# LilYau350/Variance-Aware-Weight

Hardware: AMD Instinct MI355X
Metric: training images/sec (higher is better)
Workload: dtype bf16; 1 GPU; DiT-B/4, 4x32x32 latents, 1000 classes; Trainer.train_step: q_sample + fwd + lambda-weighted MSE + bwd + AdamW + EMA; global batch 256 = 256 per GPU; global_batch=256, per_gpu_batch=256, parallelism=dp1, weight_type=lambda, hip_graph=False

## Files before the change

include/vaw_hip.h:

```cpp
#ifndef VAW_HIP_H
#define VAW_HIP_H
#include <stdint.h>

#ifdef __cplusplus
extern "C" {
#endif

typedef enum { VAW_OK = 0, VAW_ERR_INVALID = -1, VAW_ERR_LAUNCH = -2, VAW_ERR_UNSUPPORTED = -3 } vaw_status;
typedef enum { VAW_F32 = 0, VAW_BF16 = 1,
               VAW_FP8 = 2, VAW_BF8 = 3 ,
               VAW_F64 = 4  } vaw_dtype;
typedef void* vaw_stream;

int vaw_version(void);
const char* vaw_last_error_string(void);


int vaw_qsample_fwd(const float* x0, const float* noise, const int64_t* t, const float* tab_a, const float* tab_s,
                    int num_timesteps, float* x_t, int B, int64_t per_sample, vaw_stream stream);

int vaw_mix_rows(const float* x, const float* y, const float* ca, const float* cb, float* out, int B,
                 int64_t per_sample, vaw_stream stream);

int vaw_wmse_fwd(const float* model_out, const float* x0, const float* noise, const float* ca, const float* cb,
// ... 95 lines not shown
                        vaw_stream stream);


#define VAW_RESAMPLER_MAX_T 4096

int vaw_resampler_update(const int64_t* ts, const float* losses, int n, int T, int H, double* ring, int64_t* seen, int* bad,
                         vaw_stream stream);

int vaw_resampler_draw(const double* ring, const int64_t* seen, int T, int H, double uniform_prob, const double* u, int B,
                       int64_t* out_t, float* out_w, double* p, vaw_stream stream);


int vaw_row_sqnorms(const float* X, int64_t n, int D, float* out, vaw_stream stream);

int64_t vaw_pairwise_workspace_bytes(int64_t nu, int64_t nv, int k1);
int vaw_pairwise_ksmallest(const float* U, int64_t nu, const float* V, int64_t nv, int D, const float* norm_u, const float* norm_v,
                           int k1, float* out, void* ws, int64_t ws_bytes, vaw_stream stream);

int vaw_ksmallest_merge(const float* parts, int64_t n, int P, int k1, int64_t part_stride, int64_t row_stride, float* out,
                        vaw_stream stream);

int vaw_pairwise_within(const float* U, int64_t nu, const float* V, int64_t nv, int D, const float* norm_u, const float* norm_v,
                        const float* radii_u, int Ku, const float* radii_v, int Kv, uint8_t* u_in, uint8_t* v_in, vaw_stream stream);

int64_t vaw_pairwise_polysum_workspace_bytes(int64_t nu, int64_t nv, int batches);
int vaw_pairwise_polysum(const float* U, int64_t nu, const float* V, int64_t nv, int D, const int32_t* u_idx, const int32_t* v_idx, int batches,
                         double gamma, double coef0, int degree, int skip_diagonal, double* rowsum, void* ws, int64_t ws_bytes,
                         vaw_stream stream);

int64_t vaw_pairwise_count_workspace_bytes(int64_t nu, int64_t nv, int Kv);
int vaw_pairwise_count_within(const float* U, int64_t nu, const float* V, int64_t nv, int D, const float* norm_u, const float* norm_v,
                              const float* radii_v, int Kv, int32_t* u_count, uint8_t* v_in, void* ws, int64_t ws_bytes, vaw_stream stream);

int vaw_col_mean_f64(const float* X, int64_t n, int D, double* mu, vaw_stream stream);
int vaw_cov_f64(const float* X, int64_t n, int D, const double* mu, double* sigma, vaw_stream stream);

int vaw_head_logits(const float* X, int64_t n, int D, const float* Wt, int C, float* logits, int64_t ld, vaw_stream stream);
int vaw_is_rows(const float* in, int64_t n, int C, int64_t ld, int probs, double* lse, double* h, vaw_stream stream);
int vaw_is_colsums(const float* in, const double* lse, int64_t n, int C, int64_t ld, int probs, int64_t row0, int64_t split_size, double* colsum,
                   vaw_stream stream);
int vaw_is_finish(const double* h, const double* colsum, int64_t N, int C, int64_t split_size, double* scores, vaw_stream stream);


typedef struct {
    const float* bias;
    int act;
    const void* aux_in;
    void* aux_out;
    const float* gate;
    int64_t gate_ld;
    const void* resid;
    const float* rowadd;
    int rows_per_batch;
    float alpha;
    float beta;
    int out_f32;
    float* colsum_out;
    float colsum_beta;
    int resid_is_act;
    float* rowsum_a_out;
    float rowsum_a_beta;
    float* colsum_partial_out;
    int64_t* colsum_rows_out;
} vaw_epilogue;

int vaw_gemm(vaw_dtype dt, int a_kmajor, int b_kmajor, int64_t M, int64_t N, int64_t K, const void* A, int64_t lda,
             const void* B, int64_t ldb, void* C, int64_t ldc, const vaw_epilogue* epi_host, float* workspace,
             int64_t workspace_floats, vaw_stream stream);

typedef struct {
    const void* dy;
    const void* x;
    float* dw;
    int64_t M, N, ld_dy, ld_x, ld_dw;
    float alpha;
    int pad_;
    const float* scale_dy;
    const float* scale_x;
} vaw_wgrad_problem;
int64_t vaw_wgrad_grouped_desc_bytes(int n_problems);
int vaw_wgrad_grouped(vaw_dtype dt, int n_problems, const vaw_wgrad_problem* problems, int64_t K, float beta, void* desc_dev,
                      int upload, float* workspace, int64_t workspace_floats, vaw_stream stream);
void vaw_debug_wgrad_engine(int mode);

int64_t vaw_fp8_quantize_workspace_floats(void);
int vaw_fp8_quantize(vaw_dtype src_dt, vaw_dtype dst_format, const void* src, int64_t R, int64_t C, int64_t ld, void* q, int64_t ldq,
                     void* qt, int64_t ldt, float* scale_out, float* workspace, int64_t workspace_floats, vaw_stream stream);
int vaw_fp8_quantize_delayed(vaw_dtype src_dt, vaw_dtype dst_format, const void* src, int64_t R, int64_t C, int64_t ld, void* q,
                             int64_t ldq, void* qt, int64_t ldt, float* state, vaw_stream stream);
int vaw_fp8_scale_update(float* states, int64_t n, vaw_stream stream);
typedef struct {
    const float* src;
    void* q;
    void* qt;
    float* state;
    int64_t R, C, ld, ldq, ldt;
} vaw_fp8_quant_job;
int64_t vaw_fp8_quantize_batched_desc_bytes(int n_jobs);
int vaw_fp8_quantize_delayed_batched(int n_jobs, const vaw_fp8_quant_job* jobs, void* desc_dev, int upload, vaw_stream stream);
int vaw_gemm_fp8(vaw_dtype a_format, int64_t M, int64_t N, int64_t K, const void* A, int64_t lda, const float* scale_a,
                 const void* B, int64_t ldb, const float* scale_b, void* C, int64_t ldc, const vaw_epilogue* epi_host,
                 float* c_fp8_state, vaw_dtype c_fp8_format, float* workspace, int64_t workspace_floats, vaw_stream stream);
int vaw_fp8_transpose(const void* q, int64_t R, int64_t C, int64_t ldq, void* qt, int64_t ldt, vaw_stream stream);

void vaw_p8_set_reserved_cus(int n);
int vaw_gemm_uses_bf16_mfma(vaw_dtype dt, int64_t M, int64_t N, int64_t K, const void* A, int64_t lda, const void* B,
                            int64_t ldb);

typedef struct {
    int tile;
    int force_generic;
    int bk;
    int pd, ws;
    int xcdsplit;
    int sm_max_m, sm_wide_m, sm_nb, sm_stages;
    int ws_loaders;
    int epi, debug;
    int p8_nt, nt_aux;
    int cus;
} vaw_gemm_knobs;
void vaw_gemm_default_knobs(vaw_gemm_knobs* out);
typedef enum {
    VAW_GV_GENERIC = 0,
    VAW_GV_T128_BK32 = 1,
    VAW_GV_T128_BK64 = 2,
    VAW_GV_RING256 = 3,
    VAW_GV_PERSISTENT = 4,
    VAW_GV_SMALL_M = 5,
    VAW_GV_PARKED_DRAIN = 6,
    VAW_GV_WARP_SPEC = 7
} vaw_gemm_variant;
typedef enum { VAW_GR_NONE = 0, VAW_GR_F32 = 1, VAW_GR_BF16 = 2, VAW_GR_F32_ROWSUM = 3 } vaw_gemm_reduce;
typedef enum { VAW_GS_NONE = 0, VAW_GS_FUSED = 1, VAW_GS_SEPARATE = 2 } vaw_gemm_rowsum_mode;
typedef enum { VAW_GC_NONE = 0, VAW_GC_FOLD = 1, VAW_GC_DEFERRED = 2, VAW_GC_SEPARATE = 3 } vaw_gemm_colsum_mode;
typedef struct {
    int variant;
    int ntw;
    int mb, nb, stages;
    int bkt;
    int epi_kind;
    int split;
    int xcd_parts;
    int grid_x, grid_y, grid_z, block;
    int64_t lds_bytes;
    int reduce;
    int rowsum_mode;
    int colsum_mode;
    int64_t colsum_rows;
    int64_t workspace_floats_used;
    int launches;
    int status;
} vaw_gemm_launch;
int vaw_gemm_plan(vaw_dtype dt, int a_kmajor, int b_kmajor, int64_t M, int64_t N, int64_t K, int64_t lda, int64_t ldb,
                  int64_t ldc, int64_t A, int64_t B, int64_t C, const vaw_epilogue* epi_host, int64_t workspace_floats,
                  const vaw_gemm_knobs* knobs, vaw_gemm_launch* out);

typedef struct {
    int epi_kind;
    int a_e5m2;
    int c_fp8, c_e5m2;
    int ntw;
    int tiles_m, tiles_n;
    int nk;
    int split;
    int grid, block;
    int64_t lds_bytes;
// ... 137 lines not shown

int64_t vaw_groupnorm_workspace_floats(int B, int HW, int C);
int vaw_groupnorm_fwd(vaw_dtype dt, const void* x, const float* gamma, const float* beta, const float* scale,
                      const float* shift, int64_t film_ld, int silu, void* y, float* mean, float* rstd, int B, int HW,
                      int C, int G, float eps, float* workspace, vaw_stream stream);
int vaw_groupnorm_apply(vaw_dtype dt, const void* x, const float* mean, const float* rstd, const float* gamma,
                        const float* beta, const float* scale, const float* shift, int64_t film_ld, int silu, void* y, int B,
                        int HW, int C, int G, vaw_stream stream);
int vaw_groupnorm_bwd(vaw_dtype dt, const void* dout, const void* x, const float* mean, const float* rstd,
                      const float* gamma, const float* beta, const float* scale, const float* shift, int64_t film_ld,
                      int silu, const void* dx_add, void* dx, float* dgamma, float* dbeta, float grad_beta, float* dscale,
                      float* dshift, int64_t dfilm_ld, int B, int HW, int C, int G, float* workspace, vaw_stream stream);
typedef enum { VAW_GN_FWD_SUMS = 0, VAW_GN_APPLY = 1, VAW_GN_BWD_SUMS = 2, VAW_GN_BWD_APPLY = 3 } vaw_gn_pass;
typedef enum {
    VAW_GNV_QUAD = 0,
    VAW_GNV_FLAT = 1
} vaw_gn_variant;
typedef struct {
    int variant;
    int rows, nch;
    int nt, rpi;
    int grid_x, grid_y, grid_z, block;
    int64_t lds_bytes;
    int64_t workspace_floats;
    int64_t off_part, off_sums, off_s1, off_s2;
    int status;
} vaw_gn_launch;
int vaw_gn_plan(int pass, vaw_dtype dt, int B, int HW, int C, int G, vaw_gn_launch* out);
int vaw_im2col3x3(vaw_dtype dt, const void* x, void* col, int B, int H, int W, int C, vaw_stream stream);
int vaw_col2im3x3(vaw_dtype dt, const void* dcol, void* dx, int B, int H, int W, int C, vaw_stream stream);
int vaw_conv3x3(vaw_dtype dt, int mode, const void* act, const void* act2, const void* w, void* out, int B, int H, int W,
                int Ci, int Co, const vaw_epilogue* epi_host, float* workspace, int64_t workspace_floats, vaw_stream stream);
typedef enum { VAW_CVR_NONE = 0, VAW_CVR_F32 = 1, VAW_CVR_F32_ROWSUM = 2, VAW_CVR_SLAB_T = 3 } vaw_conv_reduce;
typedef enum { VAW_CVB_NONE = 0, VAW_CVB_FUSED = 1, VAW_CVB_FOLD = 2, VAW_CVB_SEPARATE = 3 } vaw_conv_bias_grad;
typedef struct {
    int variant;
    int ntw;
    int epi_kind;
    int transposed;
    int64_t M, N, K;
    int split;
    int xcd_parts;
    int grid_x, grid_y, block;
    int64_t lds_bytes;
    int reduce;
    int bias_grad;
    int colsum_mode;
    int64_t colsum_rows;
    int64_t workspace_floats_used;
    int launches;
    int status;
} vaw_conv3x3_launch;
int vaw_conv3x3_plan(vaw_dtype dt, int mode, int64_t act, int64_t act2, int64_t w, int64_t out, int B, int H, int W, int Ci, int Co,
                     const vaw_epilogue* epi_host, int64_t workspace, int64_t workspace_floats, const vaw_gemm_knobs* knobs, int cus,
                     vaw_conv3x3_launch* plan);
int64_t vaw_conv3x3_wgrad_small_workspace_floats(int B, int H, int W, int Ci, int Co);
int vaw_conv3x3_wgrad_small(vaw_dtype dt, const void* dy, const void* x, float* dw, float beta, int B, int H, int W, int Ci,
                            int Co, float* workspace, int64_t workspace_floats, vaw_stream stream);
int vaw_resample2(vaw_dtype dt, const void* in, void* out, int B, int Ho, int Wo, int C, int mode, float s,
                  vaw_stream stream);
int vaw_concat_channels(vaw_dtype dt, void* a, void* b, void* cat, int64_t M, int Ca, int Cb, int split,
                        vaw_stream stream);
int vaw_add_inplace(vaw_dtype dt, void* dst, const void* src, int64_t n, vaw_stream stream);
int vaw_mul(vaw_dtype dt, const void* a, const void* b, void* out, int64_t n, vaw_stream stream);
int vaw_subsample2(vaw_dtype dt, const void* in, void* out, int B, int Ho, int Wo, int C, int mode, vaw_stream stream);
int64_t vaw_dropout_bits_words(int64_t n);
int vaw_dropout_pack(vaw_dtype dt, const void* mask, void* bits, int64_t M, int C, vaw_stream stream);
int vaw_dropout_bits_fwd(vaw_dtype dt, const void* x, const void* bits, float keep_scale, void* y, int64_t n, vaw_stream stream);
int vaw_dropout_bits_bwd(vaw_dtype dt, const void* dy, const void* bits, float keep_scale, void* dx, int64_t n, vaw_stream stream);
int vaw_rowvec_add(vaw_dtype dt, void* h, const float* e, int64_t ld, int B, int HW, int C, vaw_stream stream);
int vaw_rowvec_sum(vaw_dtype dt, const void* dh, float* de, int64_t ld, int B, int HW, int C, float beta, vaw_stream stream);
int vaw_nchw_to_nhwc(vaw_dtype dt, const float* nchw, void* nhwc, int B, int C, int HW, vaw_stream stream);
int vaw_nhwc_to_nchw(vaw_dtype dt, const void* nhwc, float* nchw, int B, int C, int HW, vaw_stream stream);


int64_t vaw_sumsq_workspace_floats(void);
int vaw_sumsq(const float* g, int64_t n, float* sumsq_out, int accumulate, float* workspace, vaw_stream stream);
int vaw_adamw_ema_step(float* p, float* g, float* m, float* v, float* ema, void* shadow_bf16, int64_t n, float lr,
                       float beta1, float beta2, float eps, float weight_decay, float bc1, float bc2,
                       float ema_decay, const float* sumsq, float clip_max_norm, int zero_grad, vaw_stream stream);
int vaw_adamw_ema_step_dev(float* p, float* g, float* m, float* v, float* ema, void* shadow_bf16, int64_t n,
                           const float* hyper, float beta1, float beta2, float eps, float weight_decay, float ema_decay,
                           const float* sumsq, float clip_max_norm, int zero_grad, vaw_stream stream);
int vaw_ema_update(float* ema, const float* src, int64_t n, float decay, vaw_stream stream);
int vaw_cast_bf16(const float* src, void* dst, int64_t n, vaw_stream stream);
typedef struct {
    int grid_x, block;
    int rows_per_lane;
    int64_t bytes_read, bytes_written;
} vaw_cast_colsum_launch;
int vaw_cast_colsum_plan(int64_t M, int64_t N, int64_t ld_src, int64_t ld_dst, int64_t src_addr, int64_t dst_addr,
                         int64_t colsum_addr, vaw_cast_colsum_launch* out);
int vaw_cast_colsum_bf16(const float* src, int64_t ld_src, void* dst, int64_t ld_dst, int64_t M, int64_t N, float* colsum,
                         float beta, vaw_stream stream);
int vaw_uncast_bf16(const void* src, float* dst, int64_t n, float scale, vaw_stream stream);

typedef struct {
    int records;
    int colsum_sets;
    int own_dy;
    int Bk;
    int64_t block_bytes;
    int64_t block_stat_bytes;
    int64_t shared_bytes;
    int64_t colsum_bytes;
    int64_t scratch_bytes;
    int64_t cond_bytes;
    int64_t total;
} vaw_dit_ws_plan_t;
int vaw_dit_ws_plan(int dtype, int B, int T, int D, int Dm, int depth, int heads, int Kp, int No, int defer_wgrad, int checkpoint,
                    vaw_dit_ws_plan_t* out);

int vaw_comm_unique_id(void* out128);
int vaw_comm_init(const void* id128, int rank, int world);
int vaw_comm_world(void);
int vaw_comm_destroy(void);
int vaw_allreduce_bucket_start(void* buf, int64_t count, vaw_dtype dt, vaw_stream stream);
int vaw_reduce_scatter_bucket_start(void* buf, int64_t count, vaw_dtype dt, vaw_stream stream);
int vaw_allgather_bucket_start(void* buf, int64_t count, vaw_dtype dt, vaw_stream stream);
int vaw_allreduce_bucket_wait(vaw_stream stream);

#ifdef __cplusplus
}
#endif
#endif
```

variance-aware-weight_amd/_lib.py:

```python
import ctypes as C
import os

import torch

_HERE = os.path.dirname(os.path.abspath(__file__))
LIB_PATH = os.environ.get("VAW_HIP_LIB") or os.path.join(_HERE, "libvaw_hip.so")

F32, BF16, FP8, BF8 = 0, 1, 2, 3
F64 = 4
TORCH_DTYPE = {F32: torch.float32, BF16: torch.bfloat16}

_p, _i, _l, _f, _d = C.c_void_p, C.c_int, C.c_int64, C.c_float, C.c_double


class Epilogue(C.Structure):
    _fields_ = [("bias", _p), ("act", _i), ("aux_in", _p), ("aux_out", _p), ("gate", _p), ("gate_ld", _l),
                ("resid", _p), ("rowadd", _p), ("rows_per_batch", _i), ("alpha", _f), ("beta", _f), ("out_f32", _i),
                ("colsum_out", _p), ("colsum_beta", _f), ("resid_is_act", _i), ("rowsum_a_out", _p), ("rowsum_a_beta", _f),
                ("colsum_partial_out", _p), ("colsum_rows_out", C.POINTER(C.c_int64))]


class AttnDesc(C.Structure):
    _fields_ = [("B", _i), ("H", _i), ("T", _i), ("hd", _i), ("q_sb", _l), ("q_sh", _l), ("q_st", _l), ("q_sd", _l),
                ("o_sb", _l), ("o_sh", _l), ("o_st", _l), ("o_sd", _l), ("scale", _f)]
# ... 75 lines not shown
GN_FWD_SUMS, GN_APPLY, GN_BWD_SUMS, GN_BWD_APPLY = range(4)
GNV_QUAD, GNV_FLAT = range(2)

_PROTOS = {
    "vaw_qsample_fwd": [_p, _p, _p, _p, _p, _i, _p, _i, _l, _p],
    "vaw_mix_rows": [_p, _p, _p, _p, _p, _i, _l, _p],
    "vaw_wmse_fwd": [_p, _p, _p, _p, _p, _p, _p, _i, _l, _p],
    "vaw_wmse_bwd": [_p, _p, _p, _p, _p, _p, _p, _p, _i, _l, _p],
    "vaw_gemm": [_i, _i, _i, _l, _l, _l, _p, _l, _p, _l, _p, _l, C.POINTER(Epilogue), _p, _l, _p],
    "vaw_gemm_uses_bf16_mfma": [_i, _l, _l, _l, _p, _l, _p, _l],
    "vaw_colsum": [_i, _p, _l, _l, _l, _p, _f, _p, _l, _p],
    "vaw_ln_modulate_fwd": [_i, _p, _p, _p, _l, _p, _p, _p, _i, _i, _i, _f, _p],
    "vaw_gate_resid_fwd_contracts": [_i, _i, _i],
    "vaw_gate_resid_ln_modulate_fwd": [_i, _p, _p, _l, _p, _p, _p, _p, _l, _p, _p, _p, _i, _i, _i, _f, _p],
    "vaw_ln_modulate_bwd": [_i, _p, _p, _p, _p, _p, _l, _p, _p, _p, _p, _l, _i, _i, _i, _p, _l, _p],
    "vaw_gate_bwd": [_i, _p, _p, _p, _l, _p, _p, _l, _p, _i, _i, _i, _p, _l, _p],
    "vaw_reduce_rows": [_p, _l, _l, _p, _f, _p],
    "vaw_reduce_rows_batched": [_i, _p, _f, _p, _i, _p],
    "vaw_ln_modulate_bwd_gate": [_i, _p, _p, _p, _p, _p, _l, _p, _p, _p, _p, _l, _p, _p, _p, _p, _p, _i, _i, _i, _p, _l, _p],
    "vaw_ln_modulate_bwd_gate_fp8": [_p, _p, _p, _p, _p, _l, _p, _p, _p, _p, _l, _p, _p, _p, _p, _i, _p, _p, _i, _i, _i, _p, _l, _p],
    "vaw_patchify": [_i, _p, _p, _i, _i, _i, _i, _i, _p],
    "vaw_patchify_bwd": [_p, _p, _i, _i, _i, _i, _i, _p],
    "vaw_unpatchify": [_i, _p, _p, _i, _i, _i, _i, _i, _p],
    "vaw_unpatchify_bwd": [_i, _p, _p, _i, _i, _i, _i, _i, _p],
    "vaw_timestep_embedding": [_i, _p, _p, _i, _i, _f, _p],
    "vaw_silu_fwd": [_i, _p, _p, _l, _p],
    "vaw_silu_bwd": [_p, _p, _p, _l, _p],
    "vaw_add_embedding": [_p, _p, _p, _p, _i, _i, _i, _p],
    "vaw_embedding_bwd": [_p, _p, _p, _i, _i, _i, _f, _p],
    "vaw_attn_fwd": [_i, C.POINTER(AttnDesc), _p, _p, _p, _p, _p, _p],
    "vaw_attn_bwd": [_i, C.POINTER(AttnDesc), _p, _p, _p, _p, _p, _p, _p, _p, _p, _p, _p],
    "vaw_attn_bwd_colsum": [_i, C.POINTER(AttnDesc), _p, _p, _p, _p, _p, _p, _p, _p, _p, _p, _p, C.POINTER(C.c_int64), _p],
    "vaw_comm_unique_id": [_p],
    "vaw_comm_init": [_p, _i, _i],
    "vaw_comm_world": [],
    "vaw_comm_destroy": [],
    "vaw_allreduce_bucket_start": [_p, _l, _i, _p],
    "vaw_reduce_scatter_bucket_start": [_p, _l, _i, _p],
    "vaw_allgather_bucket_start": [_p, _l, _i, _p],
    "vaw_allreduce_bucket_wait": [_p],
    "vaw_groupnorm_fwd": [_i, _p, _p, _p, _p, _p, _l, _i, _p, _p, _p, _i, _i, _i, _i, _f, _p, _p],
    "vaw_groupnorm_apply": [_i, _p, _p, _p, _p, _p, _p, _p, _l, _i, _p, _i, _i, _i, _i, _p],
    "vaw_groupnorm_bwd": [_i, _p, _p, _p, _p, _p, _p, _p, _p, _l, _i, _p, _p, _p, _p, _f, _p, _p, _l, _i, _i, _i, _i, _p, _p],
    "vaw_im2col3x3": [_i, _p, _p, _i, _i, _i, _i, _p],
    "vaw_col2im3x3": [_i, _p, _p, _i, _i, _i, _i, _p],
    "vaw_conv3x3": [_i, _i, _p, _p, _p, _p, _i, _i, _i, _i, _i, C.POINTER(Epilogue), _p, _l, _p],
    "vaw_vb_fwd": [_p, _p, _p, _p, _p, _i, _i, _f, _p, _i, _l, _p],
    "vaw_vb_bwd": [_p, _p, _p, _p, _p, _i, _i, _f, _p, _p, _p, _i, _l, _p],
    "vaw_bpd_terms": [_p, _p, _l, _p, _p, _p, _p, _i, _i, _i, _p, _p, _p, _l, _i, _i, _l, _p],
    "vaw_guided_sample_step": [_i, _p, _p, _p, _p, _l, _f, _p, _p, _p, _i, _i, _i, _f, _p, _p, _p, _p, _i, _l, _p],
    "vaw_cfg_combine": [_p, _p, _l, _f, _p, _i, _l, _p],
    "vaw_finish_images": [_p, _i, _p, _i, _i, _i, _i, _p],
    "vaw_edm_input": [_p, _p, _p, _i, _i, _p, _p, _p, _i, _l, _p],
    "vaw_edm_step": [_i, _i, _p, _p, _l, _f, _p, _p, _p, _i, _i, _p, _p, _p, _i, _l, _p],
    "vaw_dpm_input": [_p, _p, _i, _i, _p, _p, _i, _l, _p],
    "vaw_dpm_step": [_i, _i, _p, _p, _l, _f, _p, _p, _p, _p, _p, _i, _i, _p, _p, _p, _p, _i, _l, _p],
    "vaw_flow_step": [_i, _i, _i, _p, _p, _l, _f, _p, _p, _p, _p, _p, _p, _i, _i, _i, _p, _p, _i, _l, _p],
    "vaw_randn_seeded": [_p, _i, _p, _i, _l, _l, _i, _i, _p],
    "vaw_rk_stage": [_i, _i, _p, _p, _l, _f, _p, _p, _p, _i, _i, _p, C.POINTER(_i), C.POINTER(_f), _i, _f, _p, _p, _p, _f, _f, _p, _l, _i, _l, _p],
    "vaw_rk_scaled_sumsq": [_p, _p, _p, _p, _f, _f, _p, _l, _i, _l, _p],
    "vaw_rk_sumsq_finish": [_p, _l, _p, _p],
    "vaw_flow_logp_stage": [_i, _p, _l, _p, _p, _p, _p, _p, _i, _i, _p, _p, C.POINTER(C.c_double), _i, C.c_double, _p, _p, _p, _l, _i, _l, _p],
    "vaw_flow_logp_prior": [_p, _p, _p, _l, _i, _l, _p],
    "vaw_prior_bpd": [_p, _f, _f, _p, _i, _l, _p],
    "vaw_resampler_update": [_p, _p, _i, _i, _i, _p, _p, _p, _p],
    "vaw_resampler_draw": [_p, _p, _i, _i, C.c_double, _p, _i, _p, _p, _p, _p],
    "vaw_conv3x3_narrow": [_i, _i, _p, _p, _p, _p, _i, _i, _i, _i, _i, _p],
    "vaw_conv3x3_wgrad_small": [_i, _p, _p, _p, _f, _i, _i, _i, _i, _i, _p, _l, _p],
    "vaw_resample2": [_i, _p, _p, _i, _i, _i, _i, _i, _f, _p],
    "vaw_concat_channels": [_i, _p, _p, _p, _l, _i, _i, _i, _p],
    "vaw_add_inplace": [_i, _p, _p, _l, _p],
    "vaw_mul": [_i, _p, _p, _p, _l, _p],
    "vaw_subsample2": [_i, _p, _p, _i, _i, _i, _i, _i, _p],
    "vaw_dropout_pack": [_i, _p, _p, _l, _i, _p],
    "vaw_dropout_bits_fwd": [_i, _p, _p, _f, _p, _l, _p],
    "vaw_dropout_bits_bwd": [_i, _p, _p, _f, _p, _l, _p],
    "vaw_rowvec_add": [_i, _p, _p, _l, _i, _i, _i, _p],
    "vaw_rowvec_sum": [_i, _p, _p, _l, _i, _i, _i, _f, _p],
    "vaw_nchw_to_nhwc": [_i, _p, _p, _i, _i, _i, _p],
    "vaw_nhwc_to_nchw": [_i, _p, _p, _i, _i, _i, _p],
    "vaw_sumsq": [_p, _l, _p, _i, _p, _p],
    "vaw_adamw_ema_step_dev": [_p, _p, _p, _p, _p, _p, _l, _p, _f, _f, _f, _f, _f, _p, _f, _i, _p],
    "vaw_adamw_ema_step": [_p, _p, _p, _p, _p, _p, _l, _f, _f, _f, _f, _f, _f, _f, _f, _p, _f, _i, _p],
    "vaw_ema_update": [_p, _p, _l, _f, _p],
    "vaw_cast_bf16": [_p, _p, _l, _p],
    "vaw_uncast_bf16": [_p, _p, _l, _f, _p],
    "vaw_wgrad_grouped": [_i, _i, _p, _l, _f, _p, _i, _p, _l, _p],
    "vaw_fp8_quantize": [_i, _i, _p, _l, _l, _l, _p, _l, _p, _l, _p, _p, _l, _p],
    "vaw_fp8_quantize_delayed": [_i, _i, _p, _l, _l, _l, _p, _l, _p, _l, _p, _p],
    "vaw_fp8_scale_update": [_p, _l, _p],
    "vaw_fp8_quantize_delayed_batched": [_i, _p, _p, _i, _p],
    "vaw_gemm_fp8": [_i, _l, _l, _l, _p, _l, _p, _p, _l, _p, _p, _l, C.POINTER(Epilogue), _p, _i, _p, _l, _p],
    "vaw_gemm_fp8_plan": [_i, _l, _l, _l, _l, _l, _l, _l, _l, _l, _l, _l, C.POINTER(Epilogue), _l, _i, _l, _l, _i, C.POINTER(GemmFp8Launch)],
    "vaw_fp8_transpose": [_p, _l, _l, _l, _p, _l, _p],
    "vaw_ln_modulate_fwd_fp8": [_p, _p, _p, _l, _p, _p, _i, _p, _p, _i, _i, _i, _f, _p],
    "vaw_gate_bwd_fp8": [_p, _p, _p, _l, _p, _p, _i, _p, _l, _p, _i, _i, _i, _p, _l, _p],
    "vaw_row_plan": [_i, _i, _l, _l, _l, _l, _l, _l, C.POINTER(RowLaunch)],
    "vaw_attn_plan": [_i, _i, C.POINTER(AttnDesc), _l, _l, _l, _l, _l, _l, _l, C.POINTER(AttnLaunch)],
    "vaw_gn_plan": [_i, _i, _i, _i, _i, _i, C.POINTER(GnLaunch)],
    "vaw_gemm_plan": [_i, _i, _i, _l, _l, _l, _l, _l, _l, _l, _l, _l, C.POINTER(Epilogue), _l, C.POINTER(GemmKnobs), C.POINTER(GemmLaunch)],
    "vaw_conv3x3_plan": [_i, _i, _l, _l, _l, _l, _i, _i, _i, _i, _i, C.POINTER(Epilogue), _l, _l, C.POINTER(GemmKnobs), _i, C.POINTER(Conv3x3Launch)],
    "vaw_dit_ws_plan": [_i, _i, _i, _i, _i, _i, _i, _i, _i, _i, _i, C.POINTER(DitWsPlan)],
    "vaw_latent_qsample": [_p, _p, _p, _p, _p, _p, _i, _f, _f, _p, _p, _p, _i, _l, _p],
    "vaw_wmse_fwd_t": [_p, _p, _p, _p, _p, _p, _p, _i, _p, _p, _f, _i, _l, _p],
    "vaw_wmse_bwd_t": [_p, _p, _p, _p, _p, _p, _p, _i, _p, _f, _p, _i, _l, _p],
    "vaw_ln_modulate_bwd_cast": [_i, _p, _p, _p, _p, _p, _l, _p, _p, _p, _p, _l, _i, _i, _i, _p, _l, _p, _p],
    "vaw_silu_bwd_cast": [_p, _p, _p, _p, _l, _p],
    "vaw_cast_colsum_plan": [_l, _l, _l, _l, _l, _l, _l, C.POINTER(CastColsumLaunch)],
    "vaw_cast_colsum_bf16": [_p, _l, _p, _l, _l, _l, _p, _f, _p],
    "vaw_row_sqnorms": [_p, _l, _i, _p, _p],
    "vaw_pairwise_ksmallest": [_p, _l, _p, _l, _i, _p, _p, _i, _p, _p, _l, _p],
    "vaw_ksmallest_merge": [_p, _l, _i, _i, _l, _l, _p, _p],
    "vaw_pairwise_within": [_p, _l, _p, _l, _i, _p, _p, _p, _i, _p, _i, _p, _p, _p],
    "vaw_pairwise_polysum": [_p, _l, _p, _l, _i, _p, _p, _i, _d, _d, _i, _i, _p, _p, _l, _p],
    "vaw_pairwise_count_within": [_p, _l, _p, _l, _i, _p, _p, _p, _i, _p, _p, _p, _l, _p],
    "vaw_col_mean_f64": [_p, _l, _i, _p, _p],
    "vaw_cov_f64": [_p, _l, _i, _p, _p, _p],
    "vaw_head_logits": [_p, _l, _i, _p, _i, _p, _l, _p],
    "vaw_is_rows": [_p, _l, _i, _l, _i, _p, _p, _p],
    "vaw_is_colsums": [_p, _p, _l, _i, _l, _i, _l, _l, _p, _p],
    "vaw_is_finish": [_p, _p, _l, _i, _l, _p, _p],
}

_lib = None


class VawError(RuntimeError):
    pass


def lib():
    global _lib
    if _lib is None:
        if not os.path.exists(LIB_PATH):
            raise VawError(f"{LIB_PATH} not found: build it with `python -c 'import __graft_entry__ as g; g.build()'` "
                           "(there is no CPU fallback for the HIP path)")
        L = C.CDLL(LIB_PATH)
        for name, args in _PROTOS.items():
            if not hasattr(L, name) and os.environ.get("VAW_HIP_LIB"):
                continue
            fn = getattr(L, name)
            fn.argtypes = args
            fn.restype = _i
        L.vaw_version.restype = _i
        L.vaw_last_error_string.restype = C.c_char_p
        L.vaw_colsum_workspace_floats.argtypes = [_l, _l]
        L.vaw_colsum_workspace_floats.restype = _l
        L.vaw_row_bwd_workspace_floats.argtypes = [_i, _i, _i]
        L.vaw_row_bwd_workspace_floats.restype = _l
        L.vaw_conv3x3_wgrad_small_workspace_floats.argtypes = [_i, _i, _i, _i, _i]
        L.vaw_conv3x3_wgrad_small_workspace_floats.restype = _l
        L.vaw_groupnorm_workspace_floats.argtypes = [_i, _i, _i]
        L.vaw_groupnorm_workspace_floats.restype = _l
        if hasattr(L, "vaw_dropout_bits_words"):
            L.vaw_dropout_bits_words.argtypes = [_l]
            L.vaw_dropout_bits_words.restype = _l
        L.vaw_wgrad_grouped_desc_bytes.argtypes = [_i]
        L.vaw_wgrad_grouped_desc_bytes.restype = _l
        L.vaw_reduce_rows_batched_desc_bytes.argtypes = [_i]
        L.vaw_reduce_rows_batched_desc_bytes.restype = _l
        L.vaw_fp8_quantize_batched_desc_bytes.argtypes = [_i]
        L.vaw_fp8_quantize_batched_desc_bytes.restype = _l
        L.vaw_fp8_quantize_workspace_floats.argtypes = []
        L.vaw_fp8_quantize_workspace_floats.restype = _l
        if hasattr(L, "vaw_pairwise_workspace_bytes"):
            L.vaw_pairwise_workspace_bytes.argtypes = [_l, _l, _i]
            L.vaw_pairwise_workspace_bytes.restype = _l
        if hasattr(L, "vaw_pairwise_polysum_workspace_bytes"):
            L.vaw_pairwise_polysum_workspace_bytes.argtypes = [_l, _l, _i]
            L.vaw_pairwise_polysum_workspace_bytes.restype = _l
            L.vaw_pairwise_count_workspace_bytes.argtypes = [_l, _l, _i]
            L.vaw_pairwise_count_workspace_bytes.restype = _l
        if hasattr(L, "vaw_rk_partial_count"):
            L.vaw_rk_partial_count.argtypes = [_i, _l]
            L.vaw_rk_partial_count.restype = _l
        L.vaw_sumsq_workspace_floats.argtypes = []
        L.vaw_sumsq_workspace_floats.restype = _l
        L.vaw_debug_force_rowwise_attention.argtypes = [_i]
        L.vaw_debug_force_rowwise_attention.restype = None
        L.vaw_debug_force_generic_gemm.argtypes = [_i]
        L.vaw_debug_force_generic_gemm.restype = None
        L.vaw_debug_gemm_tile.argtypes = [_i]
        L.vaw_debug_gemm_tile.restype = None
        if hasattr(L, "vaw_gemm_default_knobs"):
            L.vaw_gemm_default_knobs.argtypes = [C.POINTER(GemmKnobs)]
            L.vaw_gemm_default_knobs.restype = None
        if hasattr(L, "vaw_debug_gn_flat"):
            L.vaw_debug_gn_flat.argtypes = [_i]
            L.vaw_debug_gn_flat.restype = None
        L.vaw_p8_set_reserved_cus.argtypes = [_i]
        L.vaw_p8_set_reserved_cus.restype = None
        if hasattr(L, "vaw_debug_wgrad_engine"):
            L.vaw_debug_wgrad_engine.argtypes = [_i]
            L.vaw_debug_wgrad_engine.restype = None
        L.vaw_debug_cu_hog.argtypes = [_i, _i, _p]
        L.vaw_debug_cu_hog.restype = _i
        _lib = L
    return _lib


def exported_symbols():
    return sorted(list(_PROTOS) + ["vaw_version", "vaw_last_error_string", "vaw_colsum_workspace_floats",
                                   "vaw_sumsq_workspace_floats", "vaw_groupnorm_workspace_floats", "vaw_wgrad_grouped_desc_bytes",
                                   "vaw_conv3x3_wgrad_small_workspace_floats", "vaw_row_bwd_workspace_floats",
                                   "vaw_fp8_quantize_workspace_floats", "vaw_p8_set_reserved_cus", "vaw_debug_wgrad_engine", "vaw_reduce_rows_batched_desc_bytes", "vaw_fp8_quantize_batched_desc_bytes",
                                   "vaw_gemm_default_knobs", "vaw_dropout_bits_words", "vaw_pairwise_workspace_bytes", "vaw_rk_partial_count",
                                   "vaw_pairwise_polysum_workspace_bytes", "vaw_pairwise_count_workspace_bytes"])


STEP_FUSED = os.environ.get("VAW_STEP_FUSED", "1") != "0"
ROWS_FWD_FUSED = os.environ.get("VAW_ROWS_FWD_FUSED", "1") != "0"


def check(rc, what):
    if rc != 0:
        raise VawError(f"{what} failed ({rc}): {lib().vaw_last_error_string().decode()}")


def stream_ptr():
    return torch.cuda.current_stream().cuda_stream


def ptr(t):
    return 0 if t is None else t.data_ptr()


def need_cuda(*tensors):
    for t in tensors:
        if t is not None and not t.is_cuda:
            raise VawError("vaw_amd runs on the GPU only: got a CPU tensor (no CPU fallback exists by design)")
```

variance-aware-weight_amd/csrc/elementwise.hip:

```cpp
#include "common.h"

static inline int stream_grid(int64_t work_items, int block) {
    int64_t g = (work_items + block - 1) / block;
    const int64_t cap = 256 * 8;
    return (int)(g < 1 ? 1 : (g > cap ? cap : g));
}

__device__ __forceinline__ void gather_mix_coef(const float* __restrict__ ca, const float* __restrict__ cb, const int64_t* __restrict__ t,
                                                int T, int b, float& a, float& c) {
    const int64_t tt = t[b];
    const bool ok = tt >= 0 && tt < T;
    a = ok ? ca[tt] : __builtin_nanf("");
    c = ok ? cb[tt] : __builtin_nanf("");
}

template <bool GATHER>
__global__ void mix_rows_kernel(const float* __restrict__ x, const float* __restrict__ y, const float* __restrict__ ca,
                                const float* __restrict__ cb, const int64_t* __restrict__ t, int T,
                                float* __restrict__ out, int64_t n) {
    const int b = blockIdx.y;
    float a, c;
    if (GATHER) {
        gather_mix_coef(ca, cb, t, T, b, a, c);
    } else {
// ... 776 lines not shown

__device__ __forceinline__ void adam_one(float& p, float& g, float& m, float& v, float& e, bool has_ema, float gs,
                                         const AdamArgs& a) {
    const float gg = g * gs;
    p = p * (1.f - a.lr * a.wd);
    m = m + (gg - m) * (1.f - a.b1);
    v = v * a.b2 + (1.f - a.b2) * gg * gg;
    const float denom = sqrtf(v) / a.bc2_sqrt + a.eps;
    p = p - (a.lr / a.bc1) * (m / denom);
    if (has_ema) e = e * a.ema_decay + p * (1.f - a.ema_decay);
}

#define ADAM_U 4
__device__ __forceinline__ f32x4 nt_load4(const float* p) { return __builtin_nontemporal_load(reinterpret_cast<const f32x4*>(p)); }
__global__ void __launch_bounds__(256)
adamw_ema_kernel(float* __restrict__ p, float* __restrict__ g, float* __restrict__ m, float* __restrict__ v,
                 float* __restrict__ ema, bf16_t* __restrict__ shadow, int64_t n, const float* __restrict__ sumsq, AdamArgs a,
                 const float* __restrict__ hyper) {
    if (hyper) {
        a.lr = hyper[0];
        a.bc1 = hyper[1];
        a.bc2_sqrt = sqrtf(hyper[2]);
    }
    float gs = 1.f;
    if (a.clip > 0.f) {
        const float coef = a.clip / (sqrtf(*sumsq) + 1e-6f);
        gs = coef < 1.f ? coef : 1.f;
    }
    const int64_t n4 = n / 4;
    const bool has_ema = ema != nullptr;
    constexpr int64_t TILE = (int64_t)ADAM_U * 256;
    const int64_t n_tiles = n4 / TILE;
    for (int64_t t = blockIdx.x; t < n_tiles; t += gridDim.x) {
        const int64_t i0 = t * TILE + threadIdx.x;
        f32x4 pv[ADAM_U], gv[ADAM_U], mv[ADAM_U], vv[ADAM_U], ev[ADAM_U];
#pragma unroll
        for (int u = 0; u < ADAM_U; ++u) {
            const int64_t i = 4 * (i0 + 256 * u);
            pv[u] = nt_load4(p + i); gv[u] = nt_load4(g + i); mv[u] = nt_load4(m + i); vv[u] = nt_load4(v + i);
            ev[u] = has_ema ? nt_load4(ema + i) : f32x4{0, 0, 0, 0};
        }
#pragma unroll
        for (int u = 0; u < ADAM_U; ++u) {
            const int64_t i = 4 * (i0 + 256 * u);
#pragma unroll
            for (int j = 0; j < 4; ++j) {
                float pj = pv[u][j], gj = gv[u][j], mj = mv[u][j], vj = vv[u][j], ej = ev[u][j];
                adam_one(pj, gj, mj, vj, ej, has_ema, gs, a);
                pv[u][j] = pj; mv[u][j] = mj; vv[u][j] = vj; ev[u][j] = ej;
            }
            __builtin_nontemporal_store(pv[u], reinterpret_cast<f32x4*>(p + i));
            __builtin_nontemporal_store(mv[u], reinterpret_cast<f32x4*>(m + i));
            __builtin_nontemporal_store(vv[u], reinterpret_cast<f32x4*>(v + i));
            if (has_ema) __builtin_nontemporal_store(ev[u], reinterpret_cast<f32x4*>(ema + i));
            if (shadow) store4(shadow + i, pv[u]);
            if (a.zero_grad) store4(g + i, f32x4{0, 0, 0, 0});
        }
    }
    for (int64_t i = n_tiles * TILE + blockIdx.x * (int64_t)blockDim.x + threadIdx.x; i < n4; i += (int64_t)gridDim.x * blockDim.x) {
        f32x4 pv = load4(p + 4 * i), gv = load4(g + 4 * i), mv = load4(m + 4 * i), vv = load4(v + 4 * i);
        f32x4 ev = has_ema ? load4(ema + 4 * i) : f32x4{0, 0, 0, 0};
#pragma unroll
        for (int j = 0; j < 4; ++j) {
            float pj = pv[j], gj = gv[j], mj = mv[j], vj = vv[j], ej = ev[j];
            adam_one(pj, gj, mj, vj, ej, has_ema, gs, a);
            pv[j] = pj; mv[j] = mj; vv[j] = vj; ev[j] = ej;
        }
        store4(p + 4 * i, pv);
        store4(m + 4 * i, mv);
        store4(v + 4 * i, vv);
        if (has_ema) store4(ema + 4 * i, ev);
        if (shadow) store4(shadow + 4 * i, pv);
        if (a.zero_grad) store4(g + 4 * i, f32x4{0, 0, 0, 0});
    }
    for (int64_t i = n4 * 4 + blockIdx.x * (int64_t)blockDim.x + threadIdx.x; i < n; i += (int64_t)gridDim.x * blockDim.x) {
        float pv = p[i], gv = g[i], mv = m[i], vv = v[i], ev = has_ema ? ema[i] : 0.f;
        adam_one(pv, gv, mv, vv, ev, has_ema, gs, a);
        p[i] = pv; m[i] = mv; v[i] = vv;
        if (has_ema) ema[i] = ev;
        if (shadow) shadow[i] = (bf16_t)pv;
        if (a.zero_grad) g[i] = 0.f;
    }
}
static inline int adam_grid(int64_t n) {
    const int64_t tiles = n / 4 / (ADAM_U * 256);
    const int64_t cap = 256 * 8;
    return (int)(tiles < 1 ? 1 : (tiles > cap ? cap : tiles));
}

extern "C" int vaw_adamw_ema_step(float* p, float* g, float* m, float* v, float* ema, void* shadow_bf16, int64_t n,
                                  float lr, float beta1, float beta2, float eps, float weight_decay, float bc1,
                                  float bc2, float ema_decay, const float* sumsq, float clip_max_norm, int zero_grad,
                                  vaw_stream stream) {
    VAW_CHECK_ARG(n > 0, "adamw: n<=0");
    VAW_CHECK_ARG((((uintptr_t)p | (uintptr_t)g | (uintptr_t)m | (uintptr_t)v | (uintptr_t)ema) & 15) == 0 &&
                      ((uintptr_t)shadow_bf16 & 7) == 0, "adamw: buffers must be 16-byte aligned");
    VAW_CHECK_ARG(clip_max_norm <= 0.f || sumsq != nullptr, "adamw: clip needs sumsq");
    AdamArgs a{lr, beta1, beta2, eps, weight_decay, bc1, sqrtf(bc2), ema_decay, clip_max_norm, zero_grad};
    adamw_ema_kernel<<<adam_grid(n), 256, 0, (hipStream_t)stream>>>(p, g, m, v, ema, (bf16_t*)shadow_bf16, n, sumsq, a, nullptr);
    VAW_CHECK_LAUNCH("adamw_ema");
    return VAW_OK;
}

extern "C" int vaw_adamw_ema_step_dev(float* p, float* g, float* m, float* v, float* ema, void* shadow_bf16, int64_t n,
                                      const float* hyper, float beta1, float beta2, float eps, float weight_decay,
                                      float ema_decay, const float* sumsq, float clip_max_norm, int zero_grad,
                                      vaw_stream stream) {
    VAW_CHECK_ARG(n > 0 && hyper, "adamw_dev: n<=0 or no hyper buffer");
    VAW_CHECK_ARG((((uintptr_t)p | (uintptr_t)g | (uintptr_t)m | (uintptr_t)v | (uintptr_t)ema) & 15) == 0 &&
                      ((uintptr_t)shadow_bf16 & 7) == 0, "adamw_dev: buffers must be 16-byte aligned");
    VAW_CHECK_ARG(clip_max_norm <= 0.f || sumsq != nullptr, "adamw_dev: clip needs sumsq");
    AdamArgs a{0.f, beta1, beta2, eps, weight_decay, 1.f, 1.f, ema_decay, clip_max_norm, zero_grad};
    adamw_ema_kernel<<<adam_grid(n), 256, 0, (hipStream_t)stream>>>(p, g, m, v, ema, (bf16_t*)shadow_bf16, n, sumsq, a, hyper);
    VAW_CHECK_LAUNCH("adamw_ema_dev");
    return VAW_OK;
}

__global__ void ema_kernel(float* __restrict__ ema, const float* __restrict__ src, int64_t n, float d) {
    for (int64_t i = blockIdx.x * (int64_t)blockDim.x + threadIdx.x; i < n; i += (int64_t)gridDim.x * blockDim.x)
        ema[i] = ema[i] * d + src[i] * (1.f - d);
}
extern "C" int vaw_ema_update(float* ema, const float* src, int64_t n, float decay, vaw_stream stream) {
    VAW_CHECK_ARG(n > 0, "ema: n<=0");
    ema_kernel<<<stream_grid(n, 256), 256, 0, (hipStream_t)stream>>>(ema, src, n, decay);
    VAW_CHECK_LAUNCH("ema");
    return VAW_OK;
}

__global__ void cast_bf16_kernel(const float* __restrict__ src, bf16_t* __restrict__ dst, int64_t n) {
    const int64_t n4 = n / 4;
    for (int64_t i = blockIdx.x * (int64_t)blockDim.x + threadIdx.x; i < n4; i += (int64_t)gridDim.x * blockDim.x)
        store4(dst + 4 * i, load4(src + 4 * i));
    for (int64_t i = n4 * 4 + blockIdx.x * (int64_t)blockDim.x + threadIdx.x; i < n; i += (int64_t)gridDim.x * blockDim.x)
        dst[i] = (bf16_t)src[i];
}
extern "C" int vaw_cast_bf16(const float* src, void* dst, int64_t n, vaw_stream stream) {
    VAW_CHECK_ARG(n > 0 && ((uintptr_t)src & 15) == 0 && ((uintptr_t)dst & 7) == 0, "cast_bf16: n<=0 or unaligned");
    cast_bf16_kernel<<<stream_grid(n / 4 + 1, 256), 256, 0, (hipStream_t)stream>>>(src, (bf16_t*)dst, n);
    VAW_CHECK_LAUNCH("cast_bf16");
    return VAW_OK;
}

__global__ void uncast_bf16_kernel(const bf16_t* __restrict__ src, float* __restrict__ dst, int64_t n, float scale) {
    const int64_t n8 = n / 8;
    for (int64_t i = blockIdx.x * (int64_t)blockDim.x + threadIdx.x; i < n8; i += (int64_t)gridDim.x * blockDim.x) {
        const bf16x8 v = reinterpret_cast<const bf16x8*>(src)[i];
        f32x4 a = {(float)v[0], (float)v[1], (float)v[2], (float)v[3]}, b = {(float)v[4], (float)v[5], (float)v[6], (float)v[7]};
        reinterpret_cast<f32x4*>(dst)[2 * i] = a * scale;
        reinterpret_cast<f32x4*>(dst)[2 * i + 1] = b * scale;
    }
    for (int64_t i = n8 * 8 + blockIdx.x * (int64_t)blockDim.x + threadIdx.x; i < n; i += (int64_t)gridDim.x * blockDim.x)
        dst[i] = scale * (float)src[i];
}
extern "C" int vaw_uncast_bf16(const void* src, float* dst, int64_t n, float scale, vaw_stream stream) {
    VAW_CHECK_ARG(n > 0 && ((uintptr_t)src & 15) == 0 && ((uintptr_t)dst & 15) == 0, "uncast_bf16: n<=0 or unaligned");
    uncast_bf16_kernel<<<stream_grid(n / 8 + 1, 256), 256, 0, (hipStream_t)stream>>>((const bf16_t*)src, dst, n, scale);
    VAW_CHECK_LAUNCH("uncast_bf16");
    return VAW_OK;
}

__global__ void latent_qsample_kernel(const float* __restrict__ latent, const float* __restrict__ eps, const float* __restrict__ noise,
                                      const int64_t* __restrict__ t, const float* __restrict__ tab_a, const float* __restrict__ tab_s,
                                      int T, float scale, float t_scale, float* __restrict__ x0, float* __restrict__ x_t,
                                      float* __restrict__ tf, int64_t n) {
    const int b = blockIdx.y;
    float a, c;
    gather_mix_coef(tab_a, tab_s, t, T, b, a, c);
    if (tf && blockIdx.x == 0 && threadIdx.x == 0) tf[b] = (float)t[b] * t_scale;
    const float* mr = latent + (int64_t)b * 2 * n;
    const float* sr = mr + n;
    const float* er = eps + (int64_t)b * n;
    const float* nr = noise + (int64_t)b * n;
    float* xr = x0 + (int64_t)b * n;
    float* orow = x_t + (int64_t)b * n;
    const int64_t n4 = ((n & 3) == 0) ? n / 4 : 0;
    for (int64_t i = blockIdx.x * (int64_t)blockDim.x + threadIdx.x; i < n4; i += (int64_t)gridDim.x * blockDim.x) {
        const f32x4 x = (load4(mr + 4 * i) + load4(sr + 4 * i) * load4(er + 4 * i)) * scale;
        store4(xr + 4 * i, x);
        store4(orow + 4 * i, a * x + c * load4(nr + 4 * i));
    }
    for (int64_t i = n4 * 4 + blockIdx.x * (int64_t)blockDim.x + threadIdx.x; i < n; i += (int64_t)gridDim.x * blockDim.x) {
        const float x = (mr[i] + sr[i] * er[i]) * scale;
        xr[i] = x;
        orow[i] = a * x + c * nr[i];
    }
}

extern "C" int vaw_latent_qsample(const float* latent, const float* eps, const float* noise, const int64_t* t, const float* tab_a,
                                  const float* tab_s, int num_timesteps, float latent_scale, float t_scale, float* x0, float* x_t,
                                  float* t_float, int B, int64_t per_sample, vaw_stream stream) {
    VAW_CHECK_ARG(B > 0 && B <= 65535 && per_sample > 0 && num_timesteps > 0, "latent_qsample: bad sizes B=%d n=%ld", B, (long)per_sample);
    VAW_CHECK_ARG(latent && eps && noise && t && tab_a && tab_s && x0 && x_t, "latent_qsample: null pointer");
    VAW_CHECK_ARG(per_sample % 4 != 0 || ((((uintptr_t)latent | (uintptr_t)eps | (uintptr_t)noise | (uintptr_t)x0 | (uintptr_t)x_t) & 15) == 0),
                  "latent_qsample: tensors must be 16-byte aligned");
    int gx = stream_grid(per_sample / 4 + 1, 256);
    dim3 grid(gx > 64 ? 64 : gx, B);
    latent_qsample_kernel<<<grid, 256, 0, (hipStream_t)stream>>>(latent, eps, noise, t, tab_a, tab_s, num_timesteps, latent_scale, t_scale,
// ... 100 lines not shown
```

variance-aware-weight_amd/csrc/gemm_p8.hip:

```cpp
#include "gemm_p8_kernel.h"
#include "gemm_plan.h"
static_assert(P8Cfg<3>::lds_bytes == vaw_lds_p8(3) && P8Cfg<4>::lds_bytes == vaw_lds_p8(4), "gemm_plan.h: LDS size of the persistent kernel");

void p8_launch_fwd(const P8Launch& L, const EpiDev& e, hipStream_t s);
void p8_launch_dgrad(const P8Launch& L, const EpiDev& e, hipStream_t s);
void p8_launch_wgrad(const P8Launch& L, const EpiDev& e, hipStream_t s);
void p8_launch_tn(const P8Launch& L, const EpiDev& e, hipStream_t s);

static int g_p8_reserved = 0;
extern "C" void vaw_p8_set_reserved_cus(int n) { g_p8_reserved = n > 0 ? n : 0; }
static int p8_num_cus() {
    static int n = 0, env_r = 0;
    if (!n) {
        int dev = 0;
        hipDeviceProp_t prop;
        if (hipGetDevice(&dev) == hipSuccess && hipGetDeviceProperties(&prop, dev) == hipSuccess) n = prop.multiProcessorCount;
        if (n <= 0) n = 256;
        const char* v = getenv("VAW_P8_RESERVE_CUS");
        env_r = v ? atoi(v) : 0;
    }
    const int r = env_r > g_p8_reserved ? env_r : g_p8_reserved;
    return (r > 0 && r < n - 8) ? n - r : n;
}

int vaw_p8_cus_available() { return p8_num_cus(); }

static double p8_cost(int64_t M, int64_t N, int ntw, int split, int cus) {
    const int bn = 64 * ntw;
    const int64_t items = ((M + 255) / 256) * ((N + bn - 1) / bn) * split;
    const int64_t rounds = (items + cus - 1) / cus;
    return (double)rounds * (ntw == 4 ? 1.0 : 0.85) / split;
}

P8Plan vaw_p8_plan(int64_t M, int64_t N, int64_t K, bool plain_f32, bool want_colsum, int64_t ws_floats, int force, int cus) {
    P8Plan pl{false, 4, 1, 0};
    if (force == 0) return pl;
    const int nk = (int)(K / 64);
    double best = 1e30;
    for (int ntw = 4; ntw >= 3; --ntw) {
        if (force == 2 && ntw != 4) continue;
        if (force == 3 && ntw != 3) continue;
        const int bn = 64 * ntw;
        const int64_t tiles = ((M + 255) / 256) * ((N + bn - 1) / bn);
        if (ntw == 3 && force != 3) {
            const int64_t pad4 = ((N + 255) / 256) * 256, pad3 = ((N + 191) / 192) * 192;
            if (pad3 > pad4) continue;
        }
        int smax = 1;
        if (plain_f32 && !want_colsum && ws_floats > 0) {
            int64_t s = nk / 4;
            if (s > ws_floats / (M * N)) s = ws_floats / (M * N);
            if (s > 64) s = 64;
            if (s > cus / tiles) s = cus / tiles;
            smax = s < 1 ? 1 : (int)s;
        }
        for (int s = 1; s <= smax; ++s) {
            const int per = (nk + s - 1) / s;
            if ((nk + per - 1) / per != s) continue;
            double c = p8_cost(M, N, ntw, s, cus) * nk;
            if (s > 1) c += 3.0;
            if (c < best - 1e-9) { best = c; pl.ntw = ntw; pl.split = s; }
        }
    }
    const int bn = 64 * pl.ntw;
    const int64_t items = ((M + 255) / 256) * ((N + bn - 1) / bn) * pl.split;
    pl.grid = (int)(items < cus ? items : cus);
    pl.use = force > 0 || (items >= cus / 2 && nk / pl.split >= 4 && M >= 256 && N >= 128);
    return pl;
}

void vaw_p8_launch(const P8Plan& pl, int epi, int a_kmajor, int b_kmajor, int64_t M, int64_t N, int64_t K, const bf16_t* a, int64_t lda,
                   const bf16_t* b, int64_t ldb, const EpiDev& e, hipStream_t s) {
    const int bn = 64 * pl.ntw;
    const int tiles_m = (int)((M + 255) / 256), tiles_n = (int)((N + bn - 1) / bn), nk = (int)(K / 64);
    static int team_pct = -1;
    if (team_pct < 0) { const char* v = getenv("VAW_P8_TEAM_PCT"); team_pct = v ? atoi(v) : 0; }
    const int64_t items = (int64_t)tiles_m * tiles_n * pl.split;
    const int nk_item = (nk + pl.split - 1) / pl.split;
    const int team_delay = (team_pct > 0 && items >= 2 * pl.grid) ? (int)(nk_item * 160LL * pl.ntw / 4 * team_pct / 100) : 0;
    P8Launch L{a, b, lda, ldb, nk, tiles_m, tiles_n, pl.split, pl.grid, pl.ntw, epi, team_delay};
    if (a_kmajor && b_kmajor) p8_launch_fwd(L, e, s);
    else if (a_kmajor && !b_kmajor) p8_launch_dgrad(L, e, s);
    else if (!a_kmajor && !b_kmajor) p8_launch_wgrad(L, e, s);
    else p8_launch_tn(L, e, s);
}

#include <vector>

void vaw_p8_group_fp8(int ntw, bool a_e5m2, int nk, int grid, const EpiDev& e, const P8Prob* probs_dev, const P8Group& grp, hipStream_t s);
void vaw_g4_launch_group(int nk, int grid, const EpiDev& e, const P8Prob* probs_dev, const P8Group& grp, hipStream_t s);

#define G4_BY_SHAPE 1
static int g_wgrad_engine = -2;
static int wgrad_engine() {
    if (g_wgrad_engine == -2) {
        const char* v = getenv("VAW_WGRAD_ENGINE");
        const int m = v ? atoi(v) : -1;
        g_wgrad_engine = (m == 0 || m == 1) ? m : -1;
    }
    return g_wgrad_engine;
}
extern "C" void vaw_debug_wgrad_engine(int mode) { g_wgrad_engine = (mode == 0 || mode == 1) ? mode : -1; }

extern "C" int64_t vaw_wgrad_grouped_desc_bytes(int n_problems) { return (int64_t)n_problems * (int64_t)sizeof(P8Prob); }

extern "C" int vaw_wgrad_grouped(vaw_dtype dt, int n_problems, const vaw_wgrad_problem* problems, int64_t K, float beta,
                                 void* desc_dev, int upload, float* workspace, int64_t workspace_floats, vaw_stream stream) {
    VAW_CHECK_ARG(dt == VAW_BF16 || dt == VAW_FP8 || dt == VAW_BF8, "wgrad_grouped: bf16 or fp8 operands (the f32 parity mode runs vaw_gemm per layer)");
    const bool f8 = dt == VAW_FP8 || dt == VAW_BF8;
    const int kt = f8 ? 128 : 64;
    VAW_CHECK_ARG(n_problems > 0 && problems && desc_dev && K > 0 && K % kt == 0, "wgrad_grouped: bad arguments (K %% %d)", kt);
    bool all192 = true, any_not256 = false;
    for (int i = 0; i < n_problems; ++i) {
        const vaw_wgrad_problem& q = problems[i];
        VAW_CHECK_ARG(q.dy && q.x && q.dw && q.M >= 16 && q.N >= 16 && q.M % 8 == 0 && q.N % 8 == 0, "wgrad_grouped: problem %d: M, N", i);
        if (f8) VAW_CHECK_ARG(q.ld_dy >= K && q.ld_x >= K && q.ld_dw >= q.N && q.ld_dy % 16 == 0 && q.ld_x % 16 == 0 && q.ld_dw % 4 == 0,
                              "wgrad_grouped: problem %d: leading dimensions (fp8: dy^T [M][K], x^T [N][K])", i);
        else VAW_CHECK_ARG(q.ld_dy >= q.M && q.ld_x >= q.N && q.ld_dw >= q.N && q.ld_dy % 8 == 0 && q.ld_x % 8 == 0 && q.ld_dw % 4 == 0,
                           "wgrad_grouped: problem %d: leading dimensions", i);
        VAW_CHECK_ARG((((uintptr_t)q.dy | (uintptr_t)q.x | (uintptr_t)q.dw) & 15) == 0, "wgrad_grouped: problem %d: alignment", i);
        VAW_CHECK_ARG(q.M < (1 << 30) && q.N < (1 << 30), "wgrad_grouped: problem %d too large", i);
        all192 = all192 && q.N % 192 == 0;
        any_not256 = any_not256 || q.N % 256 != 0;
    }
    const int ntw = (all192 && any_not256) ? 3 : 4, bn = 64 * ntw;
    static thread_local std::vector<P8Prob> host;
    host.resize(n_problems);
    int64_t t_total = 0;
    for (int i = 0; i < n_problems; ++i) {
        const vaw_wgrad_problem& q = problems[i];
        P8Prob& h = host[i];
        h.a = (const bf16_t*)q.dy; h.b = (const bf16_t*)q.x; h.c = q.dw;
        h.lda = q.ld_dy; h.ldb = q.ld_x; h.ldc = q.ld_dw;
        h.M = (int)q.M; h.N = (int)q.N;
        h.alpha = q.alpha != 0.f ? q.alpha : 1.f;
        h.pad_ = 0;
        h.scale_a = f8 ? q.scale_dy : nullptr;
        h.scale_b = f8 ? q.scale_x : nullptr;
        h.tiles_n = (int)((q.N + bn - 1) / bn);
        h.tile0 = (int)t_total;
        t_total += ((q.M + 255) / 256) * h.tiles_n;
        VAW_CHECK_ARG(t_total < (1 << 30), "wgrad_grouped: too many tiles");
    }
    hipStream_t s = (hipStream_t)stream;
    if (upload) {
        const hipError_t rc = vaw_upload_table(desc_dev, host.data(), sizeof(P8Prob) * n_problems, s);
        VAW_CHECK_ARG(rc == hipSuccess, "wgrad_grouped: descriptor upload failed: %s", hipGetErrorString(rc));
    }
    const int cus = p8_num_cus(), nk = (int)(K / kt);
    P8Group grp{};
    grp.n_prob = n_problems;
    grp.t_full = (int)(t_total / cus) * cus;
    grp.t_rem = (int)(t_total - grp.t_full);
    grp.n_split = 1;
    grp.slab = workspace;
    if (grp.t_rem > 0) {
        int64_t sp = cus / grp.t_rem;
        if (sp > nk / 4) sp = nk / 4;
        const int64_t per_split = (int64_t)grp.t_rem * 256 * bn;
        if (workspace_floats <= 0 || !workspace) sp = 0;
        else if (sp > workspace_floats / per_split) sp = workspace_floats / per_split;
        if (sp < 2) {
            grp.t_full = (int)t_total;
            grp.t_rem = 0;
        } else {
            const int per = (nk + (int)sp - 1) / (int)sp;
            grp.n_split = (nk + per - 1) / per;
        }
    }
    const int64_t items = grp.t_full + (int64_t)grp.t_rem * grp.n_split;
    const int grid = (int)(items < cus ? items : cus);
    EpiDev e{};
    e.alpha = 1.f;
    e.beta = beta;
    e.out_f32 = 1;
    e.rpb = 1;
    e.nt_off = 1;
    {
        static int dbg = -1;
        if (dbg < 0) { const char* v = getenv("VAW_GEMM_DEBUG"); dbg = v ? atoi(v) : 0; }
        e.debug = dbg;
    }
    if (f8) vaw_p8_group_fp8(ntw, dt == VAW_BF8, nk, grid, e, (const P8Prob*)desc_dev, grp, s);
    else if (ntw == 4) {
        const int eng = wgrad_engine();
        if (eng == 1 || (eng < 0 && G4_BY_SHAPE)) vaw_g4_launch_group(nk, grid, e, (const P8Prob*)desc_dev, grp, s);
        else p8_launch_group<4>(nk, grid, e, (const P8Prob*)desc_dev, grp, s);
    } else p8_launch_group<3>(nk, grid, e, (const P8Prob*)desc_dev, grp, s);
    if (grp.t_rem > 0) {
        if (ntw == 4) p8_group_fixup_kernel<256><<<grp.t_rem * 8, 256, 0, s>>>((const P8Prob*)desc_dev, grp, beta);
        else p8_group_fixup_kernel<192><<<grp.t_rem * 8, 256, 0, s>>>((const P8Prob*)desc_dev, grp, beta);
    }
    VAW_CHECK_LAUNCH("wgrad_grouped");
    return VAW_OK;
}
```

variance-aware-weight_amd/csrc/gemm_p8_kernel.h:

```cpp
#pragma once
#include <stdlib.h>

#include "gemm_epi.h"

typedef __attribute__((address_space(3))) void* lds_ptr_t;
typedef const __attribute__((address_space(1))) void* gbl_ptr_t;

#ifdef P8_TIMING
#define P8_TS(v) const uint64_t v = __builtin_readcyclecounter()
#define P8_TACC(tA, tB, tC, tD, tE)                                                                       \
    do { tacc[0] += tB - tA; tacc[1] += tC - tB; tacc[2] += tD - tC; tacc[3] += tE - tD; tacc[5] += 1;     \
         if (tprev) tacc[4] += tA - tprev; tprev = tE; } while (0)
#else
#define P8_TS(v) do { } while (0)
#define P8_TACC(tA, tB, tC, tD, tE) do { } while (0)
#endif

#ifndef P8_LATE_AT
#define P8_LATE_AT 2
#endif
#ifndef P8_PH2
#define P8_PH2 0
#endif
#ifndef P8_EPI_PD
// ... 768 lines not shown
    }
    if (NOBR) asm volatile("s_waitcnt vmcnt(0)" ::: "memory");
#ifdef P8_TIMING
    if (blockIdx.x == 0 && lane == 0 && (wid == 0 || wid == 4)) {
        __builtin_amdgcn_s_waitcnt(0);
        uint64_t* out = reinterpret_cast<uint64_t*>((char*)e.C + (int64_t)(wid == 4 ? 128 : 0) * e.ldc * (e.out_f32 ? 4 : 2));
        for (int i = 0; i < 6; ++i) out[i] = tacc[i];
    }
#endif
}


template <bool AK, bool BKM, int NTW, int EPI, int CONV>
static void p8_launch_conv(const bf16_t* a, int64_t lda, const bf16_t* b, int64_t ldb, int nk, int tiles_m, int tiles_n, int split,
                           int grid, const EpiDev& e, const P8Conv& cg, hipStream_t s) {
    static bool attr_done = false;
    const int lds = P8Cfg<NTW>::lds_bytes;
    if (!attr_done) {
        (void)hipFuncSetAttribute((const void*)gemm_p8_kernel<AK, BKM, NTW, EPI, false, CONV>, hipFuncAttributeMaxDynamicSharedMemorySize, lds);
        attr_done = true;
    }
    gemm_p8_kernel<AK, BKM, NTW, EPI, false, CONV><<<grid, 512, lds, s>>>(a, lda, b, ldb, nk, tiles_m, tiles_n, split, e, 0, nullptr, P8Group{}, cg);
}

template <int NTW, int EPI, int F8>
static void p8_launch_fp8_one(const void* a, int64_t lda, const void* b, int64_t ldb, int nk, int tiles_m, int tiles_n, int split, int grid,
                              const EpiDev& e, hipStream_t s) {
    static bool attr_done = false;
    const int lds = P8Cfg<NTW>::lds_bytes;
    if (!attr_done) {
        (void)hipFuncSetAttribute((const void*)gemm_p8_kernel<true, true, NTW, EPI, false, 0, F8>, hipFuncAttributeMaxDynamicSharedMemorySize, lds);
        attr_done = true;
    }
    gemm_p8_kernel<true, true, NTW, EPI, false, 0, F8><<<grid, 512, lds, s>>>((const bf16_t*)a, lda, (const bf16_t*)b, ldb, nk, tiles_m, tiles_n,
                                                                               split, e, 0, nullptr, P8Group{}, P8Conv{});
}

template <bool AK, bool BKM, int NTW, int EPI>
static void p8_launch_one(const bf16_t* a, int64_t lda, const bf16_t* b, int64_t ldb, int nk, int tiles_m, int tiles_n, int split,
                          int grid, const EpiDev& e, hipStream_t s, int team_delay) {
    static bool attr_done = false;
    const int lds = P8Cfg<NTW>::lds_bytes;
    if (!attr_done) {
        (void)hipFuncSetAttribute((const void*)gemm_p8_kernel<AK, BKM, NTW, EPI, false, 0>, hipFuncAttributeMaxDynamicSharedMemorySize, lds);
        attr_done = true;
    }
    gemm_p8_kernel<AK, BKM, NTW, EPI, false, 0><<<grid, 512, lds, s>>>(a, lda, b, ldb, nk, tiles_m, tiles_n, split, e, team_delay);
}

template <int NTW, int F8 = 0>
static void p8_launch_group(int nk, int grid, const EpiDev& e, const P8Prob* probs_dev, const P8Group& grp, hipStream_t s) {
    static bool attr_done = false;
    const int lds = P8Cfg<NTW>::lds_bytes;
    if (!attr_done) {
        (void)hipFuncSetAttribute((const void*)gemm_p8_kernel<F8 != 0, F8 != 0, NTW, P8_WGRAD, true, 0, F8>, hipFuncAttributeMaxDynamicSharedMemorySize, lds);
        attr_done = true;
    }
    gemm_p8_kernel<F8 != 0, F8 != 0, NTW, P8_WGRAD, true, 0, F8><<<grid, 512, lds, s>>>(nullptr, 0, nullptr, 0, nk, 0, 0, 1, e, 0, probs_dev, grp, P8Conv{});
}

template <int BN>
__global__ void p8_group_fixup_kernel(const P8Prob* __restrict__ probs, P8Group grp, float beta) {
    const int r = blockIdx.x >> 3, band = blockIdx.x & 7, g = grp.t_full + r;
    int pi = 0;
    while (pi + 1 < grp.n_prob && probs[pi + 1].tile0 <= g) ++pi;
    const P8Prob pr = probs[pi];
    const int tile = g - pr.tile0, tm = tile / pr.tiles_n, tn = tile - tm * pr.tiles_n;
    const int64_t m0 = (int64_t)tm * P8_BM + 32 * band, n0 = (int64_t)tn * BN;
    constexpr int C4 = BN / 4;
    for (int i = threadIdx.x; i < 32 * C4; i += blockDim.x) {
        const int row = i / C4, c4 = (i - row * C4) * 4;
        const int64_t m = m0 + row, n = n0 + c4;
        if (m >= pr.M || n >= pr.N) continue;
        f32x4 acc = {0, 0, 0, 0};
        for (int sp = 0; sp < grp.n_split; ++sp)
            acc += load4(grp.slab + ((int64_t)sp * grp.t_rem + r) * (P8_BM * BN) + (int64_t)(32 * band + row) * BN + c4);
        float* c = pr.c + m * pr.ldc + n;
        acc *= pr.alpha * (pr.scale_a ? *pr.scale_a : 1.f) * (pr.scale_b ? *pr.scale_b : 1.f);
        if (beta != 0.f) acc += beta * load4(c);
        store4(c, acc);
    }
}

struct P8Launch {
    const bf16_t *a, *b;
    int64_t lda, ldb;
    int nk, tiles_m, tiles_n, split, grid, ntw, epi, team_delay;
};
#define P8_CASE(AKv, BKv, EPIv)                                                                                                  \
    case EPIv:                                                                                                                  \
        if (L.ntw == 4) p8_launch_one<AKv, BKv, 4, EPIv>(L.a, L.lda, L.b, L.ldb, L.nk, L.tiles_m, L.tiles_n, L.split, L.grid, e, s, L.team_delay); \
        else p8_launch_one<AKv, BKv, 3, EPIv>(L.a, L.lda, L.b, L.ldb, L.nk, L.tiles_m, L.tiles_n, L.split, L.grid, e, s, L.team_delay);           \
        break
```

variance-aware-weight_amd/dit.py:

```python
import os

import numpy as np
import torch
import torch.nn as nn

from . import _lib as L
from . import ops
from ._lib import BF16, F32, ptr
from .flat import FlatModule

__all__ = ["DiT", "DiT_S", "DiT_B", "DiT_L", "DiT_XL", "DiT_models"]


def _sincos_1d(dim, pos):
    omega = 1.0 / 10000 ** (np.arange(dim // 2, dtype=np.float64) / (dim / 2.0))
    ang = np.einsum("m,d->md", pos.reshape(-1), omega)
    return np.concatenate([np.sin(ang), np.cos(ang)], axis=1)


def get_2d_sincos_pos_embed(dim, grid_size):
    gh = np.arange(grid_size, dtype=np.float32)
    gw = np.arange(grid_size, dtype=np.float32)
    grid = np.stack(np.meshgrid(gw, gh), axis=0).reshape([2, 1, grid_size, grid_size])
    return np.concatenate([_sincos_1d(dim // 2, grid[0]), _sincos_1d(dim // 2, grid[1])], axis=1)
# ... 130 lines not shown
            cps = dict(fc2=ops.ColsumPartial(B, D, dev), proj=ops.ColsumPartial(B, D, dev),
                       fc1=ops.ColsumPartial((M + 63) // 64, m.Dm, dev), qkv=ops.ColsumPartial(max(B, M // 64), 3 * D, dev))
            cps["fc2"].rows.value = cps["proj"].rows.value = B
            self._bufs += [c.buf for c in cps.values()]
            return cps

        self.cp = [cp_set()] * Lyr if ckpt else [cp_set() for _ in range(Lyr)]
        if not (ckpt and plan.own_dy):
            self.dyb = e(M, D)
        self.delta = e(B * m.num_heads * T, dtype=f32)
        self.dmod, self.dmod_a = e(B, m.mod_cols, dtype=f32), z(m.mod_cols)
        self.dcs, self.dc, self.dc_a = e(B, D, dtype=f32), e(B, D, dtype=f32), z(D)
        self.dh1s, self.dh1, self.dh1_a = e(B, D, dtype=f32), e(B, D, dtype=f32), z(D)
        self.dxp = e(M, m.Kp, dtype=f32)
        if not self.fp8 and self.nbytes() != plan.total:
            raise L.VawError(f"DiT workspace: allocated {self.nbytes()} bytes, vaw_dit_ws_plan says {plan.total}")

    def nbytes(self):
        return sum(t.numel() * t.element_size() for t in self._bufs)


class _DiTFn(torch.autograd.Function):
    @staticmethod
    def forward(ctx, anchor, model, x, t, y):
        out = model._forward_impl(x, t, y)
        ctx.model, ctx.gen, ctx.need_dx = model, model._ws_cur.gen, x.requires_grad
        ctx.only_dx = bool(model._input_grad_only)
        ctx.x_shape = x.shape
        return out

    @staticmethod
    def backward(ctx, dout):
        m = ctx.model
        if m._ws_cur.gen != ctx.gen:
            raise L.VawError("DiT backward: activations were overwritten by a later forward of the same batch size")
        if m._ws_cur.ckpt != bool(m.activation_checkpointing):
            raise L.VawError("DiT backward: activation_checkpointing was switched between this forward and its backward "
                             "(the workspace of the forward was laid out for the other mode)")
        if bool(m._input_grad_only) != ctx.only_dx:
            raise L.VawError("DiT backward: input_grad_only() was entered or left between this forward and its backward")
        dx = m._backward_impl(dout.contiguous(), ctx.need_dx, ctx.only_dx)
        return (None if L.STEP_FUSED else torch.zeros_like(m._anchor)), None, dx, None, None


class DiT(FlatModule):
    def __init__(self, image_size=32, patch_size=2, in_channels=4, hidden_size=1152, depth=28, num_heads=16,
                 mlp_ratio=4.0, class_dropout_prob=0.1, num_classes=1000, learn_sigma=False, learn_align=False,
                 encoder_depth=8, z_dims=768, projector_dim=2048, compute_dtype="bf16", activation_checkpointing=False):
        super().__init__()
        if learn_align:
            raise NotImplementedError("learn_align (REPA feature alignment) is outside the hot path (SURVEY §2.1 row 12)")
        assert hidden_size % num_heads == 0 and hidden_size % 4 == 0
        self.learn_sigma, self.learn_align = learn_sigma, learn_align
        self.in_channels = in_channels
        self.out_channels = in_channels * 2 if learn_sigma else in_channels
        self.patch_size, self.num_heads, self.depth = patch_size, num_heads, depth
        self.image_size = image_size
        self.encoder_depth = encoder_depth
        self.x_embedder = _PatchEmbed(image_size, patch_size, in_channels, hidden_size)
        self.t_embedder = _TimestepEmbedder(hidden_size)
        self.y_embedder = _LabelEmbedder(num_classes, hidden_size, class_dropout_prob)
        self.pos_embed = nn.Parameter(torch.zeros(1, self.x_embedder.num_patches, hidden_size), requires_grad=False)
        self.blocks = nn.ModuleList([_Block(hidden_size, num_heads, mlp_ratio) for _ in range(depth)])
        self.projectors = None
        self.final_layer = _FinalLayer(hidden_size, patch_size, self.out_channels)
        self.initialize_weights()
        self.D, self.T = hidden_size, self.x_embedder.num_patches
        self.Dm = int(hidden_size * mlp_ratio)
        self.Kp = in_channels * patch_size * patch_size
        self.No = patch_size * patch_size * self.out_channels
        self.mod_cols = (6 * depth + 2) * hidden_size
        self.fp8_grad_format = "e5m2"
        self.fp8_scaling, self.fp8_margin = "delayed", 2.0
        self.fp8_fuse_epilogue = os.environ.get("VAW_FP8_FUSE", "1") != "0"
        self.fp8_fuse_rows = os.environ.get("VAW_FP8_FUSE_ROWS", "1") != "0"
        self._fp8_w, self._fp8_epoch, self._fp8_wstates, self._fp8_wgroup = {}, None, None, None
        self.activation_checkpointing = False
        self.set_compute_dtype(compute_dtype)
        self._anchor = torch.zeros(1, requires_grad=True)
        self._ws, self._ws_cur = {}, None
        self.set_activation_checkpointing(activation_checkpointing)
        self._ckpt_debug_hook = None
        self.grad_ready_hook = None
        self.defer_wgrad = True

    def initialize_weights(self):
        def basic(mod):
            if isinstance(mod, nn.Linear):
                nn.init.xavier_uniform_(mod.weight)
                if mod.bias is not None:
                    nn.init.constant_(mod.bias, 0)
        self.apply(basic)
        pe = get_2d_sincos_pos_embed(self.pos_embed.shape[-1], int(self.x_embedder.num_patches ** 0.5))
        self.pos_embed.data.copy_(torch.from_numpy(pe).float().unsqueeze(0))
        w = self.x_embedder.proj.weight.data
        nn.init.xavier_uniform_(w.view([w.shape[0], -1]))
        nn.init.constant_(self.x_embedder.proj.bias, 0)
        nn.init.normal_(self.y_embedder.embedding_table.weight, std=0.02)
        nn.init.normal_(self.t_embedder.mlp[0].weight, std=0.02)
        nn.init.normal_(self.t_embedder.mlp[2].weight, std=0.02)
        for blk in self.blocks:
            nn.init.constant_(blk.adaLN_modulation[-1].weight, 0)
            nn.init.constant_(blk.adaLN_modulation[-1].bias, 0)
        nn.init.constant_(self.final_layer.adaLN_modulation[-1].weight, 0)
        nn.init.constant_(self.final_layer.adaLN_modulation[-1].bias, 0)
        nn.init.constant_(self.final_layer.linear.weight, 0)
        nn.init.constant_(self.final_layer.linear.bias, 0)

    def set_compute_dtype(self, name):
        name = {"float32": "fp32", "f32": "fp32", "bfloat16": "bf16", "float8": "fp8"}.get(name, name)
        if name not in ("bf16", "fp32", "fp8"):
            raise ValueError(f"compute_dtype must be 'bf16', 'fp32' or 'fp8', got {name}")
        if name == "fp8" and (self.D % 128 or self.Dm % 128):
            raise ValueError("compute_dtype='fp8' needs hidden and MLP widths that are multiples of 128 (one fp8 MFMA K tile)")
        if name == "fp8" and getattr(self, "activation_checkpointing", False):
            raise ValueError(self._CKPT_FP8)
        if name != getattr(self, "compute_dtype", name):
            self.require_fresh_masters("set_compute_dtype()")
        self.compute_dtype = name
        self._dt = F32 if name == "fp32" else BF16
        self._fp8 = name == "fp8"
        self._fp8_w, self._fp8_epoch, self._fp8_wstates, self._fp8_wgroup = {}, None, None, None
        self._ws = {}

    _ONLY_DX_FP8 = ("input_grad_only() does not combine with compute_dtype='fp8': the delayed-scaling state of the fp8 tensors would "
                    "move during an evaluation")

    _CKPT_FP8 = ("activation_checkpointing does not combine with compute_dtype='fp8': re-running a block's forward would update its "
                 "delayed-scaling state twice per step, and the per-block transposed fp8 copies would have to be shared too")

    def set_activation_checkpointing(self, on):
        on = bool(on)
        if on and self._fp8:
            raise ValueError(self._CKPT_FP8)
        self.activation_checkpointing = on
        self._ws = {}

    def _flat_groups(self):
        ada_w = [f"blocks.{i}.adaLN_modulation.1.weight" for i in range(self.depth)] + ["final_layer.adaLN_modulation.1.weight"]
        ada_b = [f"blocks.{i}.adaLN_modulation.1.bias" for i in range(self.depth)] + ["final_layer.adaLN_modulation.1.bias"]
        return [ada_w, ada_b]

    def _apply(self, fn, recurse=True):
        r = super()._apply(fn, recurse)
        self._anchor = fn(self._anchor.detach()).requires_grad_(True)
        self._ws = {}
        return r

    def grad_stage_bounds(self):
        self.ensure_flat()
        off = lambda n: self._flat_offsets[n][0]
        first = [off(f"blocks.{l}.attn.qkv.weight") for l in range(self.depth)] + [off("final_layer.linear.weight")]
        b = {self.depth + 1: (first[-1], self._flat_n_train), 0: (0, first[0])}
        for l in range(self.depth):
            b[l + 1] = (first[l], first[l + 1])
        half = self._ada_split_block()
        if half is not None:
            D = self.D
            wo, bo = off("blocks.0.adaLN_modulation.1.weight"), off("blocks.0.adaLN_modulation.1.bias")
            we = sum(self._flat_offsets["final_layer.adaLN_modulation.1.weight"])
            be = sum(self._flat_offsets["final_layer.adaLN_modulation.1.bias"])
            assert we - wo == (6 * self.depth + 2) * D * D and be - bo == (6 * self.depth + 2) * D
            cut_w, cut_b = wo + 6 * half * D * D, bo + 6 * half * D
            b["ada_hi"] = [(cut_w, we), (cut_b, be)]
            lo = [(0, cut_w), (we, cut_b), (be, first[0])] if wo < bo else [(0, cut_b), (be, cut_w), (we, first[0])]
            b[0] = [r for r in lo if r[1] > r[0]]
        return b

    def _ada_split_block(self):
        return self.depth // 2 if self.depth >= 4 else None

    def unpatchify(self, x):
        c, p = self.out_channels, self.patch_size
        h = w = int(x.shape[1] ** 0.5)
        assert h * w == x.shape[1]
        x = x.float().contiguous()
        img = torch.empty(x.shape[0], c, h * p, w * p, device=x.device, dtype=torch.float32)
        L.check(L.lib().vaw_unpatchify(F32, ptr(x), ptr(img), x.shape[0], c, h * p, w * p, p, L.stream_ptr()), "vaw_unpatchify")
        return img

    def forward(self, x, t, y, **kwargs):
        L.need_cuda(x, t, y)
        if self._input_grad_only and self._fp8:
            raise ValueError(self._ONLY_DX_FP8)
        out = _DiTFn.apply(self._anchor, self, x, t, y)
        return out, None

    stagewise_weight_waits = True

    def _need(self, stage):
        z = getattr(self, "_zero", None)
        if z is not None:
            z.wait_stage(stage)

    def _w(self, name):
        o, _ = self._flat_offsets[name]
        return self._wbase + o * self._wsize

    def _g(self, name):
        o, _ = self._flat_offsets[name]
        return self._gbase + 4 * o

    def _p32(self, name):
        o, _ = self._flat_offsets[name]
        return self._flat.data_ptr() + 4 * o

    def _prepare(self, B):
        self.ensure_flat()
        if self._dt == BF16:
            sh = self.shadow_bf16()
            self._wbase, self._wsize = sh.data_ptr(), 2
        else:
            self._wbase, self._wsize = self._flat.data_ptr(), 4
        adt = L.TORCH_DTYPE[self._dt]
        if self._fp8:
            if (B * self.T) % 128:
                raise L.VawError("compute_dtype='fp8': batch * tokens must be a multiple of 128 (K tile of the weight gradients)")
            self._refresh_fp8_weights()
        key = (B, adt, self._fp8, bool(self.activation_checkpointing), bool(self.defer_wgrad))
        if key not in self._ws:
            self._ws[key] = _Workspace(self, B, adt)
        self._ws_cur = ws = self._ws[key]
        if ws.fp8:
            delayed = self.fp8_scaling == "delayed"
            ws.d_fwd, ws.d_bwd = delayed and ws.calib_fwd, delayed and ws.calib_bwd
            if ws.d_fwd or ws.d_bwd:
                ops.fp8_scale_update(ws.fp8_states)
        return ws

    _FP8_LINEARS = (("attn.qkv.", 3, 1), ("attn.proj.", 1, 1), ("mlp.fc1.", 0, 1), ("mlp.fc2.", 1, 0))

    def _refresh_fp8_weights(self):
        epoch = (self._weights_epoch, self._flat.data_ptr())
        if self._fp8_epoch == epoch:
            return
        self.require_fresh_masters("re-quantising the fp8 weights")
        dev = self._flat.device
        if self._fp8_wstates is None or self._fp8_wstates.device != dev:
            self._fp8_wstates, self._fp8_w, self._fp8_wgroup = ops.fp8_states([L.FP8] * (4 * self.depth), dev, self.fp8_margin), {}, None
        delayed = self.fp8_scaling == "delayed" and bool(self._fp8_w)
        if delayed:
            ops.fp8_scale_update(self._fp8_wstates)
            grp = getattr(self, "_fp8_wgroup", None)
            if grp is None or grp[0] != self._flat.data_ptr():
                pairs = [(self._p32(f"blocks.{l}.{nm}weight"), self._fp8_w[f"blocks.{l}.{nm}weight"])
                         for l in range(self.depth) for nm, _, _ in self._FP8_LINEARS]
                grp = self._fp8_wgroup = (self._flat.data_ptr(), ops.Fp8QuantGroup(pairs, dev))
            grp[1].launch()
            self._fp8_epoch = epoch
            return
# ... 141 lines not shown

    def _attn_desc(self, B):
        d = getattr(self, "_adesc", None)
        if d is None or d.B != B:
            d = self._adesc = ops.attn_desc_token_major(B, self.num_heads, self.T, self.D // self.num_heads)
        return d

    def _wgrad(self, dt, name, dy, x, Nw, Kw, M, beta, bias=True):
        ops.gemm(dt, 0, 0, Nw, Kw, M, dy, Nw, x, Kw, self._g(name + "weight"), Kw, beta=beta, out_f32=True,
                 rowsum_a_out=self._g(name + "bias") if bias else None, rowsum_a_beta=beta)

    def _adaln_wgrad(self, dt, ws, r0, nrows, B, beta):
        D, ld = self.D, self.mod_cols
        gw, gb = self._g("blocks.0.adaLN_modulation.1.weight") + 4 * r0 * D, self._g("blocks.0.adaLN_modulation.1.bias") + 4 * r0
        fused = False
        if dt == BF16:
            dmod_a, es = ptr(ws.dmod_a), 2
            fused = L.STEP_FUSED and ops.cast_colsum_plan(B, nrows, ld, ld, ptr(ws.dmod) + 4 * r0, dmod_a + es * r0, gb) is not None
            if fused:
                ops.cast_colsum(ptr(ws.dmod) + 4 * r0, ld, dmod_a + es * r0, ld, B, nrows, gb, beta)
            else:
                ops.cast_bf16(ws.dmod, ws.dmod_a)
        else:
            dmod_a, es = ptr(ws.dmod), 4
        ops.gemm(dt, 0, 0, nrows, D, ws.Bk, dmod_a + es * r0, ld, ptr(ws.cs), D, gw, D, beta=beta, out_f32=True)
        if not fused:
            ops.colsum(dt, dmod_a + es * r0, B, nrows, ld, gb, beta)
        return dmod_a

    def _backward_impl(self, dout, need_dx, only_dx=False):
        ws = self._ws_cur
        B = ws.B
        dt, D, T, Dm, Lyr, ld = self._dt, self.D, self.T, self.Dm, self.depth, self.mod_cols
        M, lib, st = B * T, L.lib(), L.stream_ptr()
        H = W = self.image_size
        if only_dx:
            if ws.fp8:
                raise ValueError(self._ONLY_DX_FP8)
            beta, self._gbase, hook = 0.0, None, None
        else:
            beta = 1.0 if self.grads_live() else 0.0
            self._gbase = self.flat_grads().data_ptr()
            hook = self.grad_ready_hook
        ada_half = self._ada_split_block() if hook else None
        dres, dD, dDm, dmod = ptr(ws.dres), ptr(ws.dD), ptr(ws.dDm), ptr(ws.dmod)
        mod = ptr(ws.mod)
        es = self._wsize
        defer = ws.defer and dt == BF16
        fp8 = ws.fp8
        own_dy = defer and not fp8
        ckpt = ws.ckpt
        fuse_rows = fp8 and ws.d_bwd and self.fp8_fuse_epilogue and self.fp8_fuse_rows and M % 64 == 0 and D % 128 == 0
        fuse_tail = L.STEP_FUSED and dt == BF16

        def ln_bwd_and_gate(dout_p, x_p, mean_p, rstd_p, scale_p, dres_in, dsh, dsc, nxt, dx_act=0):
            if nxt is None:
                ops.ln_modulate_bwd(dt, dout_p, x_p, mean_p, rstd_p, scale_p, ld, dres_in, dres, dsh, dsc, ld, B, T, D, dx_act=dx_act)
                return
            l2, which = nxt
            nb = ws.blk[l2]
            mo2, dmo2 = mod + 4 * (6 * l2 * D), dmod + 4 * (6 * l2 * D)
            gcol = 5 if which == "mlp" else 2
            y, cp = (nb["y2"], ws.cp[l2]["fc2"]) if which == "mlp" else (nb["y1"], ws.cp[l2]["proj"])
            if fuse_rows:
                ops.ln_modulate_bwd_gate_fp8(dout_p, x_p, mean_p, rstd_p, scale_p, ld, dres_in, dres, dsh, dsc, ld, ptr(y),
                                             mo2 + 4 * gcol * D, nb["f_dy2" if which == "mlp" else "f_dy1"], dmo2 + 4 * gcol * D,
                                             B, T, D, cp.buf.data_ptr())
            else:
                dy = ptr(nb["dy2" if which == "mlp" else "dy1"]) if own_dy else ptr(ws.dyb)
                ops.ln_modulate_bwd_gate(dt, dout_p, x_p, mean_p, rstd_p, scale_p, ld, dres_in, dres, dsh, dsc, ld, ptr(y),
                                         mo2 + 4 * gcol * D, dy, dmo2 + 4 * gcol * D, B, T, D, cp.buf.data_ptr())

        L.check(lib.vaw_unpatchify_bwd(dt, ptr(dout), ptr(ws.dotok), B, self.out_channels, H, W, self.patch_size, st), "unpatchify_bwd")
        if not only_dx:
            self._wgrad(dt, "final_layer.linear.", ptr(ws.dotok), ptr(ws.xf), self.No, D, M, beta)
        ops.gemm(dt, 1, 0, M, D, self.No, ptr(ws.dotok), self.No, self._w("final_layer.linear.weight"), D, dD, D)
        mo, dmo = mod + 4 * (6 * Lyr * D), dmod + 4 * (6 * Lyr * D)
        ln_bwd_and_gate(dD, ptr(ws.xres[2 * Lyr]), ptr(ws.meanf), ptr(ws.rstdf), mo + 4 * D, 0, dmo, dmo + 4 * D,
                        (Lyr - 1, "mlp") if (Lyr and not ckpt) else None)
        if hook:
            hook(Lyr + 1)
        pending = []
        group_cut = Lyr // 2 if (hook and Lyr >= 4) else 0

        def fold_bias(blocks, qkv_too):
            key = (blocks[0], blocks[-1], self._gbase, qkv_too)
            cps = []
            for l in blocks:
                cp, pre = ws.cp[l], f"blocks.{l}."
                names = [("fc2", "mlp.fc2."), ("fc1", "mlp.fc1."), ("proj", "attn.proj.")] + ([("qkv", "attn.qkv.")] if qkv_too else [])
                cps += [(cp[key_cp], pre + nm) for key_cp, nm in names]
            rows = tuple(int(cp.rows.value) for cp, _ in cps)
            ent = ws.bias_groups.get(key)
            if ent is None or ent[1] != rows:
                jobs = [(cp.buf.data_ptr(), self._g(nm + "bias"), r, cp.N) for (cp, nm), r in zip(cps, rows)]
                ent = ws.bias_groups[key] = (ops.ReduceGroup(jobs, dout.device), rows)
            grp = ent[0]
            grp.launch(beta)

        def flush():
            if not pending:
                return
            key = (pending[0], pending[-1], self._gbase)
            grp = ws.wgrad_groups.get(key)
            if grp is None:
                probs = []
                for l in pending:
                    b, pre = ws.blk[l], f"blocks.{l}."
                    if fp8:
                        for name, fdy, fx, Nw, Kw in ((pre + "mlp.fc2.", b["f_dy2"], b["f_a"], D, Dm), (pre + "mlp.fc1.", b["f_dhid"], b["f_xm2"], Dm, D),
                                                      (pre + "attn.proj.", b["f_dy1"], b["f_ao"], D, D), (pre + "attn.qkv.", b["f_dqkv"], b["f_xm"], 3 * D, D)):
                            probs.append((ptr(fdy.qt), ptr(fx.qt), self._g(name + "weight"), Nw, Kw, M, M, Kw, 0.0, 0, ptr(fdy.scale), ptr(fx.scale)))
                        continue
                    for name, dy, x, Nw, Kw in ((pre + "mlp.fc2.", b["dy2"], b["a"], D, Dm), (pre + "mlp.fc1.", b["dDm"], b["xm2"], Dm, D),
                                                (pre + "attn.proj.", b["dy1"], b["ao"], D, D), (pre + "attn.qkv.", b["dqkv"], b["xm"], 3 * D, D)):
                        probs.append((ptr(dy), ptr(x), self._g(name + "weight"), Nw, Kw, Nw, Kw, Kw))
                grp = ws.wgrad_groups[key] = ops.WgradGroup(probs, M, dout.device)
            grp.launch((L.BF8 if self.fp8_grad_format == "e5m2" else L.FP8) if fp8 else dt, beta)
            fold_bias(list(pending), True)
            if hook:
                for l in pending:
                    hook(l + 1)
            pending.clear()

        for l in reversed(range(Lyr)):
            b, cp, pre = ws.blk[l], ws.cp[l], f"blocks.{l}."
            mo, dmo = mod + 4 * (6 * l * D), dmod + 4 * (6 * l * D)
            xin, xmid = ptr(ws.xres[2 * l]), ptr(ws.xres[2 * l + 1])
            dy2, dhid, dy1, dq = ((ptr(b["dy2"]), ptr(b["dDm"]), ptr(b["dy1"]), ptr(b["dqkv"])) if own_dy
                                  else (ptr(ws.dyb), dDm, ptr(ws.dyb), ptr(ws.dqkv)))
            if ckpt:
                self._block_fwd(ws, l, xout=ptr(ws.xscr))
                if self._ckpt_debug_hook is not None:
                    self._ckpt_debug_hook(l, b)
                ops.gate_bwd(dt, dres, ptr(b["y2"]), mo + 4 * 5 * D, ld, dy2, dmo + 4 * 5 * D, ld, B, T, D, cp["fc2"].buf.data_ptr())
            if not defer and not only_dx:
                self._wgrad(dt, pre + "mlp.fc2.", dy2, ptr(b["a"]), D, Dm, M, beta, bias=False)
            fuse_dh = fp8 and ws.d_bwd and self.fp8_fuse_epilogue and M % 64 == 0
            self._linear_dgrad(ws, b, "f_dy2", None if fuse_rows else dy2, pre + "mlp.fc2.", M, D, Dm, b["f_dhid"].epilogue_target() if fuse_dh else dhid, act=2,
                               aux_in=ptr(b["hpre"]), colsum_partial=cp["fc1"], **({"out_fp8": b["f_dhid"]} if fuse_dh else {}))
            if not defer and not only_dx:
                self._wgrad(dt, pre + "mlp.fc1.", dhid, ptr(b["xm2"]), Dm, D, M, beta, bias=False)
            self._linear_dgrad(ws, b, "f_dhid", None if (fp8 and fuse_dh) else dhid, pre + "mlp.fc1.", M, Dm, D, dD)
            ln_bwd_and_gate(dD, xmid, ptr(b["mean2"]), ptr(b["rstd2"]), mo + 4 * 4 * D, dres, dmo + 4 * 3 * D, dmo + 4 * 4 * D, (l, "attn"))
            if not defer and not only_dx:
                self._wgrad(dt, pre + "attn.proj.", dy1, ptr(b["ao"]), D, D, M, beta, bias=False)
            self._linear_dgrad(ws, b, "f_dy1", None if fuse_rows else dy1, pre + "attn.proj.", M, D, D, ptr(ws.dao))
            q = ptr(b["qkv"])
            qkv_bias_folded = False
            if defer:
                qkv_bias_folded = ops.attn_bwd_colsum(dt, self._attn_desc(B), q, q + es * D, q + 2 * es * D, ptr(b["ao"]), ptr(ws.dao),
                                                      ptr(b["lse"]), ptr(ws.delta), dq, dq + es * D, dq + 2 * es * D, cp["qkv"])
            if not qkv_bias_folded:
                ops.attn_bwd(dt, self._attn_desc(B), q, q + es * D, q + 2 * es * D, ptr(b["ao"]), ptr(ws.dao), ptr(b["lse"]),
                             ptr(ws.delta), dq, dq + es * D, dq + 2 * es * D)
                if only_dx:
                    pass
                elif defer:
                    ops.colsum(dt, dq, M, 3 * D, 3 * D, cp["qkv"].buf.data_ptr(), 0.0, device=dout.device)
                    cp["qkv"].rows.value = 1
                else:
                    self._wgrad(dt, pre + "attn.qkv.", dq, ptr(b["xm"]), 3 * D, D, M, beta)
            self._linear_dgrad(ws, b, "f_dqkv", dq, pre + "attn.qkv.", M, 3 * D, D, dD)
            last_cast = fuse_tail and l == 0
            ln_bwd_and_gate(dD, xin, ptr(b["mean1"]), ptr(b["rstd1"]), mo + 4 * D, dres, dmo, dmo + 4 * D,
                            (l - 1, "mlp") if (l and not ckpt) else None, dx_act=ptr(ws.dao) if last_cast else 0)
            if only_dx:
                pass
            elif defer:
                pending.append(l)
                if ckpt or l == group_cut:
                    pending.reverse()
                    flush()
            else:
                fold_bias([l], False)
            if hook:
                if not defer:
                    hook(l + 1)
                if l == ada_half:
                    r0 = 6 * l * D
                    self._adaln_wgrad(dt, ws, r0, ld - r0, B, beta)
                    hook("ada_hi")
        pending.reverse()
        flush()
        if dt == BF16 and fuse_tail and Lyr:
            dx0 = ptr(ws.dao)
        elif dt == BF16:
            ops.cast_bf16(ws.dres, ws.dD)
            dx0 = dD
        else:
            dx0 = dres
        if not only_dx:
            self._wgrad(dt, "x_embedder.proj.", dx0, ptr(ws.xp), D, self.Kp, M, beta)
        dx = None
        if need_dx:
            ops.gemm(dt, 1, 0, M, self.Kp, D, dx0, D, self._w("x_embedder.proj.weight"), self.Kp, ptr(ws.dxp), self.Kp, out_f32=True)
            dx = torch.empty(B, self.in_channels, H, W, device=dout.device, dtype=torch.float32)
            L.check(lib.vaw_patchify_bwd(ptr(ws.dxp), ptr(dx), B, self.in_channels, H, W, self.patch_size, st), "patchify_bwd")
        if only_dx:
            return dx
        rows = ld if ada_half is None else 6 * ada_half * D
        dmod_a = self._adaln_wgrad(dt, ws, 0, rows, B, beta)
        ops.gemm(dt, 1, 0, B, D, ld, dmod_a, ld, self._w("blocks.0.adaLN_modulation.1.weight"), D, ptr(ws.dcs), D, out_f32=True)
        ops.silu_bwd(ws.c, ws.dcs, ws.dc, ws.dc_a[:B] if fuse_tail else None)
        ye = self.y_embedder.embedding_table
        L.check(lib.vaw_embedding_bwd(ptr(ws.dc), ptr(ws.y), self._g("y_embedder.embedding_table.weight"), B, D,
                                      ye.num_embeddings, beta, st), "embedding_bwd")
        if dt == BF16 and not fuse_tail:
            ops.cast_bf16(ws.dc, ws.dc_a)
        dc_a = ptr(ws.dc_a) if dt == BF16 else ptr(ws.dc)
        self._wgrad(dt, "t_embedder.mlp.2.", dc_a, ptr(ws.h1s), D, D, ws.Bk, beta)
        ops.gemm(dt, 1, 0, B, D, D, dc_a, D, self._w("t_embedder.mlp.2.weight"), D, ptr(ws.dh1s), D, out_f32=True)
        ops.silu_bwd(ws.h1, ws.dh1s, ws.dh1, ws.dh1_a[:B] if fuse_tail else None)
        if dt == BF16 and not fuse_tail:
            ops.cast_bf16(ws.dh1, ws.dh1_a)
        dh1_a = ptr(ws.dh1_a) if dt == BF16 else ptr(ws.dh1)
        self._wgrad(dt, "t_embedder.mlp.0.", dh1_a, ptr(ws.tfreq), D, 256, ws.Bk, beta)
        self.attach_grads()
        if fp8:
            ws.calib_bwd = True
        if hook:
            hook(0)
        return dx


_PRESETS = {"DiT-S": (384, 12, 6), "DiT-B": (768, 12, 12), "DiT-L": (1024, 24, 16), "DiT-XL": (1152, 28, 16)}


def _make(name):
    hidden, depth, heads = _PRESETS[name]

    def build(image_size, patch_size, in_channels, class_dropout_prob, num_classes, learn_sigma, **kwargs):
        return DiT(image_size=image_size, patch_size=patch_size, in_channels=in_channels, hidden_size=hidden,
                   depth=depth, num_heads=heads, class_dropout_prob=class_dropout_prob, num_classes=num_classes,
                   learn_sigma=learn_sigma, **kwargs)
    build.__name__ = name.replace("-", "_")
    return build


DiT_S, DiT_B, DiT_L, DiT_XL = (_make(n) for n in ("DiT-S", "DiT-B", "DiT-L", "DiT-XL"))
DiT_models = {"DiT-S": DiT_S, "DiT-B": DiT_B, "DiT-L": DiT_L, "DiT-XL": DiT_XL}
```

variance-aware-weight_amd/flat.py:

```python
import contextlib

import torch
import torch.nn as nn

from . import ops

_ALIGN = 64


def _round_up(n, a=_ALIGN):
    return (n + a - 1) // a * a


class FlatModule(nn.Module):

    def _flat_groups(self):
        return []

    def _flat_channels_last(self, name, p):
        return False

    @staticmethod
    def _view_as_param(buf, p, channels_last):
        if channels_last:
            co, ci, kh, kw = p.shape
            return buf.view(co, kh, kw, ci).permute(0, 3, 1, 2)
        return buf.view(p.shape)

    def _ordered_named_params(self):
        named = dict(self.named_parameters())
        order, seen = [], set()
        for group in self._flat_groups():
            for i, n in enumerate(group):
                order.append((n, i > 0))
                seen.add(n)
        order += [(n, False) for n in named if n not in seen]
        train = [(n, named[n], pk) for n, pk in order if named[n].requires_grad]
        frozen = [(n, named[n], pk) for n, pk in order if not named[n].requires_grad]
        return train, frozen

    def _build_flat(self):
        train, frozen = self._ordered_named_params()
        dev = train[0][1].device
        offs, off = {}, 0
        for n, p, packed in train:
            if not packed:
                off = _round_up(off)
            offs[n] = (off, p.numel())
            off += p.numel()
        n_train = off = _round_up(off)
        for n, p, packed in frozen:
            off = _round_up(off)
            offs[n] = (off, p.numel())
            off += p.numel()
        off = _round_up(off)
        flat = torch.zeros(off, device=dev, dtype=torch.float32)
        self._flat_cl = {}
        with torch.no_grad():
            for n, p, _ in train + frozen:
                o, k = offs[n]
                if p.dtype != torch.float32:
                    raise TypeError(f"{n}: master parameters must be float32, got {p.dtype}")
                cl = self._flat_cl[n] = bool(p.dim() == 4 and self._flat_channels_last(n, p))
                v = self._view_as_param(flat[o:o + k], p, cl)
                v.copy_(p.data)
                p.data = v
        self._flat = flat
        self._flat_offsets = offs
        self._flat_n_train = n_train
        self._flat_grad = None
        self._flat_shadow = None
        self._shadow_version = None
        self._weights_epoch = 0
        self._flat_params = [p for _, p, _ in train]
        self._flat_names = [n for n, _, _ in train]
        self._flat_dirty = False

    def _apply(self, fn, recurse=True):
        r = super()._apply(fn, recurse)
        self._flat_dirty = True
        return r

    def ensure_flat(self):
        if getattr(self, "_flat_dirty", True) or getattr(self, "_flat", None) is None:
            self._build_flat()
            return
        base = self._flat.data_ptr()
        for i in (0, -1):
            if self._flat_params[i].data_ptr() != base + 4 * self._flat_offsets[self._flat_names[i]][0]:
                self._build_flat()
                return

    def __deepcopy__(self, memo):
        cls = self.__class__
        new = cls.__new__(cls)
        memo[id(self)] = new
        import copy
        skip = {"_flat", "_flat_grad", "_flat_shadow", "_flat_params"}
        fresh = {"_ws": dict, "_ws_cur": lambda: None, "_adesc": lambda: None, "_tape": list, "_fp8_w": dict, "_fp8_epoch": lambda: None, "_fp8_wstates": lambda: None, "_fp8_wgroup": lambda: None, "_zero": lambda: None, "grad_ready_hook": lambda: None}
        for k, v in self.__dict__.items():
            new.__dict__[k] = None if k in skip else fresh[k]() if k in fresh else copy.deepcopy(v, memo)
        new._flat_dirty = True
        return new

    def flat_params(self):
        self.ensure_flat()
        return self._flat

    def flat_train(self):
        self.ensure_flat()
        return self._flat[: self._flat_n_train]

    def flat_grads(self):
        self.ensure_flat()
        if self._flat_grad is None:
            self._flat_grad = torch.zeros(self._flat_n_train, device=self._flat.device, dtype=torch.float32)
        return self._flat_grad

    def grad_view(self, name):
        o, k = self._flat_offsets[name]
        return self.flat_grads()[o:o + k]

    def attach_grads(self):
        g = self.flat_grads()
        for n, p in zip(self._flat_names, self._flat_params):
            if p.grad is None or p.grad.data_ptr() != g.data_ptr() + 4 * self._flat_offsets[n][0]:
                o, k = self._flat_offsets[n]
                p.grad = self._view_as_param(g[o:o + k], p, self._flat_cl[n])

    def grads_live(self):
        return self._flat_params[0].grad is not None

    def zero_grad_flat(self):
        for p in self._flat_params:
            p.grad = None

    _input_grad_only = False

    @contextlib.contextmanager
    def input_grad_only(self):
        if getattr(self, "compute_dtype", None) == "fp8":
            raise ValueError("input_grad_only() does not combine with compute_dtype='fp8': the delayed-scaling state of the fp8 "
                             "tensors would move during an evaluation")
        before = self._input_grad_only
        self._input_grad_only = True
        try:
            yield self
        finally:
            self._input_grad_only = before

    _master_stale = False

    def require_fresh_masters(self, what):
        if self._master_stale:
            raise RuntimeError(f"{what}: the f32 master parameters of other ranks' chunks are stale (sharded optimizer, bf16 mode) -- "
                               "call trainer.consolidate() / optimizer.consolidate() on EVERY rank first (it is a collective)")

    def state_dict(self, *args, **kwargs):
        self.require_fresh_masters("state_dict()")
        return super().state_dict(*args, **kwargs)

    def shadow_bf16(self):
        self.ensure_flat()
        ver = sum(p._version for p in self._flat_params)
        if self._flat_shadow is None:
            self._flat_shadow = torch.empty(self._flat.numel(), device=self._flat.device, dtype=torch.bfloat16)
            self._shadow_version = None
        if ver != self._shadow_version:
            self.require_fresh_masters("re-casting the bf16 shadow weights (a parameter was modified through torch)")
            ops.cast_bf16(self._flat, self._flat_shadow)
            self._shadow_version = ver
            self._weights_epoch += 1
        return self._flat_shadow

    def mark_weights_changed(self):
        self._shadow_version = None
        self._weights_epoch = getattr(self, "_weights_epoch", 0) + 1

    def mark_shadow_fresh(self):
        self._weights_epoch += 1
        if self._flat_shadow is not None:
            self._shadow_version = sum(p._version for p in self._flat_params)
# ... 1 lines not shown
```

variance-aware-weight_amd/ops.py:

```python
import ctypes as C
import math

import numpy as np
import torch

from . import _lib as L
from ._lib import BF16, F32, AttnDesc, Epilogue, check, need_cuda, ptr, stream_ptr


def dt_of(t):
    if t.dtype == torch.float32:
        return F32
    if t.dtype == torch.bfloat16:
        return BF16
    raise L.VawError(f"unsupported activation dtype {t.dtype}")


def _f32c(*ts):
    for t in ts:
        if t is not None and (t.dtype != torch.float32 or not t.is_contiguous()):
            raise L.VawError(f"expected a contiguous float32 tensor, got {t.dtype} contiguous={t.is_contiguous()}")


def qsample(x0, noise, t, tab_a, tab_s):
# ... 646 lines not shown

def q_scratch(n, device, pool=0):
    t = _q_scratch.get((device, pool))
    if t is None or t.numel() < n:
        t = _q_scratch[(device, pool)] = torch.empty(n, device=device, dtype=torch.uint8)
    return t


def gemm_fp8(M, N, K, A, lda, scale_a, B, ldb, scale_b, Cp, ldc, *, a_format=L.FP8, bias=None, act=0, aux_in=None, aux_out=None,
             gate=None, gate_ld=0, resid=None, rows_per_batch=0, alpha=1.0, out_f32=False, colsum_out=None, colsum_beta=0.0,
             out_fp8=None, colsum_partial=None):
    e = Epilogue(bias or None, act, aux_in or None, aux_out or None, gate or None, gate_ld, resid or None, None, rows_per_batch,
                 alpha, 0.0, 1 if out_f32 else 0, colsum_out or None, colsum_beta, 0, None, 0.0)
    if colsum_partial is not None:
        colsum_partial.rows.value = colsum_partial.buf.shape[0]
        e.colsum_partial_out, e.colsum_rows_out = colsum_partial.buf.data_ptr(), C.pointer(colsum_partial.rows)
    tr = gemm_trace
    if tr is not None:
        e0, e1 = tr.events()
        e0.record()
    ws_ptr, ws_n = 0, 0
    if colsum_out:
        ws = scratch_f32(torch.device("cuda", torch.cuda.current_device()), 0)
        ws_ptr, ws_n = ws.data_ptr(), ws.numel()
    check(L.lib().vaw_gemm_fp8(a_format, M, N, K, A, lda, scale_a, B, ldb, scale_b, Cp, ldc, C.byref(e),
                               out_fp8.state.data_ptr() if out_fp8 is not None else None, out_fp8.fmt if out_fp8 is not None else 0,
                               ws_ptr, ws_n, stream_ptr()), "vaw_gemm_fp8")
    if tr is not None:
        e1.record()
        nb = M * K + N * K + M * N * ((4 if out_f32 else 1 if out_fp8 is not None else 2) + (2 if aux_out else 0) + (2 if aux_in else 0) +
                                      (4 if resid else 0))
        tr.add(2, True, a_format == L.FP8, M, N, K, e0, e1, float(nb))


def gemm_fp8_plan(M, N, K, A, lda, scale_a, B, ldb, scale_b, Cp, ldc, *, a_format=L.FP8, workspace=16, workspace_floats=0, cus=0,
                  colsum_partial_rows=None, out_fp8_state=0, out_fp8_format=L.FP8, check_status=True, **epi):
    e = Epilogue(epi.get("bias") or None, epi.get("act", 0), epi.get("aux_in") or None, epi.get("aux_out") or None, epi.get("gate") or None,
                 epi.get("gate_ld", 0), epi.get("resid") or None, epi.get("rowadd") or None, epi.get("rows_per_batch", 0),
                 epi.get("alpha", 1.0), epi.get("beta", 0.0), 1 if epi.get("out_f32") else 0, epi.get("colsum_out") or None,
                 epi.get("colsum_beta", 0.0), 1 if epi.get("resid_is_act") else 0, epi.get("rowsum_a_out") or None,
                 epi.get("rowsum_a_beta", 0.0))
    rows = C.c_int64(colsum_partial_rows or 0)
    if colsum_partial_rows is not None:
        e.colsum_partial_out, e.colsum_rows_out = epi.get("colsum_partial_out", 16), C.pointer(rows)
    p = L.GemmFp8Launch()
    rc = L.lib().vaw_gemm_fp8_plan(a_format, M, N, K, A, lda, scale_a, B, ldb, scale_b, Cp, ldc, C.byref(e), out_fp8_state, out_fp8_format,
                                   workspace if workspace_floats > 0 else 0, workspace_floats, cus, C.byref(p))
    if check_status:
        check(rc, "vaw_gemm_fp8_plan")
    return p


class WgradProblem(C.Structure):
    _fields_ = [("dy", C.c_void_p), ("x", C.c_void_p), ("dw", C.c_void_p), ("M", C.c_int64), ("N", C.c_int64),
                ("ld_dy", C.c_int64), ("ld_x", C.c_int64), ("ld_dw", C.c_int64), ("alpha", C.c_float), ("pad_", C.c_int),
                ("scale_dy", C.c_void_p), ("scale_x", C.c_void_p)]


class WgradGroup:

    def __init__(self, problems, K, device):
        self.n, self.K, self.device = len(problems), int(K), device
        self.table = (WgradProblem * self.n)(*[WgradProblem(*p) for p in problems])
        self.flop = sum(2.0 * p[3] * p[4] * K for p in problems)
        self.desc = torch.empty(L.lib().vaw_wgrad_grouped_desc_bytes(self.n), device=device, dtype=torch.uint8)
        self.uploaded = False

    def launch(self, dt, beta):
        ws = scratch_f32(self.device, 0)
        tr = gemm_trace
        if tr is not None:
            e0, e1 = tr.events()
            e0.record()
        check(L.lib().vaw_wgrad_grouped(dt, self.n, C.cast(self.table, C.c_void_p), self.K, float(beta), self.desc.data_ptr(),
                                        0 if self.uploaded else 1, ws.data_ptr(), ws.numel(), stream_ptr()), "vaw_wgrad_grouped")
        self.uploaded = True
        if tr is not None:
            e1.record()
            es = 1 if dt in (L.FP8, L.BF8) else 2
            tr.add_flop(2 if dt in (L.FP8, L.BF8) else 1, False, False, self.flop, e0, e1,
                        float(sum(es * (p.M + p.N) * self.K + 4 * p.M * p.N * (2 if beta else 1) for p in self.table)))


def wgrad_engine(mode):
    L.lib().vaw_debug_wgrad_engine(int(mode))


def beta_or_plain(bias, act, aux_out, gate, resid, rowadd):
    return not (bias or act or aux_out or gate or resid or rowadd)


def conv3x3(dt, mode, act, act2, w, out, B, H, W, Ci, Co, *, bias=None, resid=None, resid_is_act=True, beta=0.0,
            colsum_out=None, colsum_beta=0.0, rowsum_a_out=None, rowsum_a_beta=0.0):
    e = Epilogue(bias or None, 0, None, None, None, 0, resid or None, None, 0, 1.0, beta, 1 if mode == 2 else 0,
                 colsum_out or None, colsum_beta, 1 if resid_is_act else 0, rowsum_a_out or None, rowsum_a_beta)
    ws = scratch_f32(torch.device("cuda", torch.cuda.current_device()), 0)
    tr = gemm_trace
    if tr is not None:
        e0, e1 = tr.events()
        e0.record()
    rc = L.lib().vaw_conv3x3(dt, mode, act, act2 or None, w, out, B, H, W, Ci, Co, C.byref(e), ws.data_ptr(), ws.numel(), stream_ptr())
    if rc == -3:
        if dt == L.BF16:
            key = ("conv3x3", ("fwd", "dgrad", "wgrad")[mode], B, H, W, Ci, Co)
            fallbacks[key] = fallbacks.get(key, 0) + 1
            if fallbacks[key] == 1:
                import warnings
                warnings.warn(f"vaw_amd: conv3x3 {key[1]} [B={B}, {H}x{W}, Ci={Ci}, Co={Co}] is not covered by the implicit-GEMM kernels "
                              "(channel counts off the 64 / 8 grid?): falling back to im2col + GEMM; counts in vaw_amd.ops.fallbacks",
                              RuntimeWarning, stacklevel=3)
        return False
    check(rc, "vaw_conv3x3")
    if tr is not None:
        e1.record()
        M = B * H * W
        nb = 2 * M * (Ci + Co) + (2 if mode != 2 else 4 * (2 if beta else 1)) * 9 * Ci * Co + ((2 * M * Co) if (mode == 0 and resid) else 0)
        tr.add(1, mode != 2, mode == 0, *((M, Co, 9 * Ci) if mode == 0 else (M, Ci, 9 * Co) if mode == 1 else (Co, 9 * Ci, M)), e0, e1, float(nb), tag=f"conv{H}x{W}")
    return True


def conv3x3_plan(dt, mode, act, act2, w, out, B, H, W, Ci, Co, *, workspace=16, workspace_floats=0, knobs=None, cus=0, check_status=True,
                 **epi):
    e = Epilogue(epi.get("bias") or None, epi.get("act", 0), None, epi.get("aux_out") or None, epi.get("gate") or None, epi.get("gate_ld", 0),
                 epi.get("resid") or None, epi.get("rowadd") or None, 0, 1.0, epi.get("beta", 0.0),
                 1 if (mode == 2 or epi.get("out_f32")) else 0, epi.get("colsum_out") or None, epi.get("colsum_beta", 0.0),
                 1 if epi.get("resid_is_act", True) else 0, epi.get("rowsum_a_out") or None, epi.get("rowsum_a_beta", 0.0))
    p = L.Conv3x3Launch()
    rc = L.lib().vaw_conv3x3_plan(dt, mode, act or 0, act2 or 0, w or 0, out or 0, B, H, W, Ci, Co, C.byref(e),
                                  workspace if workspace_floats > 0 else 0, workspace_floats, C.byref(knobs) if knobs is not None else None,
                                  cus, C.byref(p))
    if check_status:
        check(rc, "vaw_conv3x3_plan")
    return p


fallbacks = {}


class GemmTrace:

    def __init__(self):
        self.rows = []

    def events(self):
        return torch.cuda.Event(enable_timing=True), torch.cuda.Event(enable_timing=True)

    def add(self, mfma, ak, bk, M, N, K, e0, e1, nbytes=0.0, tag="gemm"):
        self.rows.append((mfma, ak, bk, 2.0 * M * N * K, e0, e1, nbytes, (tag, int(M), int(N), int(K))))

    def add_flop(self, mfma, ak, bk, flop, e0, e1, nbytes=0.0):
        self.rows.append((mfma, ak, bk, flop, e0, e1, nbytes, None))

    @staticmethod
    def _name(mfma, ak, bk):
        return ("fp8_mfma" if mfma == 2 else "bf16_mfma" if mfma else "generic_f32mfma") + ("/fwd" if ak and bk else "/dgrad" if ak else "/wgrad")

    def by_shape(self):
        acc = {}
        for mfma, ak, bk, flop, e0, e1, nbytes, shape in self.rows:
            d = acc.setdefault((self._name(mfma, ak, bk), shape), [0, 0.0, 0.0])
            d[0] += 1
            d[1] += e0.elapsed_time(e1)
            d[2] += flop
        return sorted(((k[0], k[1], v[0], v[1], v[2]) for k, v in acc.items()), key=lambda r: -r[3])

    def summarize(self):
# ... 132 lines not shown

class ReduceGroup:

    def __init__(self, jobs, device):
        self.n = len(jobs)
        self.table = (ReduceJob * self.n)(*[ReduceJob(*j) for j in jobs])
        self.desc = torch.empty(L.lib().vaw_reduce_rows_batched_desc_bytes(self.n), device=device, dtype=torch.uint8)
        self.uploaded = False

    def launch(self, beta):
        check(L.lib().vaw_reduce_rows_batched(self.n, C.cast(self.table, C.c_void_p), float(beta), self.desc.data_ptr(),
                                              0 if self.uploaded else 1, stream_ptr()), "vaw_reduce_rows_batched")
        self.uploaded = True


def gate_bwd(dt, dres, y, gate, mod_ld, dy, dgate, dmod_ld, B, T, D, dy_colpart=0):
    ws = _row_ws(B, T, D)
    check(L.lib().vaw_gate_bwd(dt, dres, y, gate, mod_ld, dy, dgate, dmod_ld, dy_colpart or None, B, T, D, ws.data_ptr(),
                               ws.numel(), stream_ptr()), "vaw_gate_bwd")


def reduce_rows(partial, R, N, out, beta):
    check(L.lib().vaw_reduce_rows(partial, R, N, out, beta, stream_ptr()), "vaw_reduce_rows")


def attn_desc_token_major(B, H, T, hd):
    return AttnDesc(B, H, T, hd, T * 3 * H * hd, hd, 3 * H * hd, 1, T * H * hd, hd, H * hd, 1, hd ** -0.5)


def attn_desc_channel_major(B, H, T, ch):
    return AttnDesc(B, H, T, ch, 3 * H * ch * T, ch * T, 1, T, H * ch * T, ch * T, 1, T, ch ** -0.5)


def attn_desc_nhwc(B, H, T, ch, new_order):
    C_ = H * ch
    desc = AttnDesc(B, H, T, ch, T * 3 * C_, ch if new_order else 3 * ch, 3 * C_, 1, T * C_, ch, C_, 1, ch ** -0.5)
    return (desc, C_, 2 * C_) if new_order else (desc, ch, 2 * ch)


def attn_plan(direction, dt, desc, q, k, v, o_or_do, dq=0, dk=0, dv=0):
    p = L.AttnLaunch()
    check(L.lib().vaw_attn_plan(direction, dt, C.byref(desc), q, k, v, o_or_do, dq, dk, dv, C.byref(p)), "vaw_attn_plan")
    return p


def dit_ws_plan(dt, B, T, D, Dm, depth, heads, Kp, No, defer_wgrad=True, checkpoint=False):
    p = L.DitWsPlan()
    check(L.lib().vaw_dit_ws_plan(dt, B, T, D, Dm, depth, heads, Kp, No, int(defer_wgrad), int(checkpoint), C.byref(p)), "vaw_dit_ws_plan")
    return p


def attn_fwd(dt, desc, q, k, v, o, lse):
    check(L.lib().vaw_attn_fwd(dt, C.byref(desc), q, k, v, o, lse, stream_ptr()), "vaw_attn_fwd")


def attn_bwd(dt, desc, q, k, v, o, d_o, lse, delta, dq, dk, dv):
    check(L.lib().vaw_attn_bwd(dt, C.byref(desc), q, k, v, o, d_o, lse, delta, dq, dk, dv, stream_ptr()), "vaw_attn_bwd")


def attn_bwd_colsum(dt, desc, q, k, v, o, d_o, lse, delta, dq, dk, dv, partial):
    partial.rows.value = partial.buf.shape[0]
    rc = L.lib().vaw_attn_bwd_colsum(dt, C.byref(desc), q, k, v, o, d_o, lse, delta, dq, dk, dv, partial.buf.data_ptr(),
                                     C.byref(partial.rows), stream_ptr())
    if rc == -3:
        return False
    check(rc, "vaw_attn_bwd_colsum")
    return True


def timestep_embedding(t, dim, dtype=torch.float32, max_period=10000.0):
    need_cuda(t)
    t = t.float().contiguous()
    out = torch.empty(t.shape[0], dim, device=t.device, dtype=dtype)
    check(L.lib().vaw_timestep_embedding(dt_of(out), ptr(t), ptr(out), t.shape[0], dim, max_period, stream_ptr()),
          "vaw_timestep_embedding")
    return out


def sumsq(g, out, accumulate=False):
    ws = scratch_f32(g.device, L.lib().vaw_sumsq_workspace_floats())
    check(L.lib().vaw_sumsq(ptr(g), g.numel(), ptr(out), 1 if accumulate else 0, ptr(ws), stream_ptr()), "vaw_sumsq")


def adamw_ema_step(p, g, m, v, ema, shadow, lr, beta1, beta2, eps, wd, step, ema_decay, sumsq_t, clip, zero_grad, hyper=None):
    if hyper is not None:
        check(L.lib().vaw_adamw_ema_step_dev(ptr(p), ptr(g), ptr(m), ptr(v), ptr(ema), ptr(shadow), p.numel(), ptr(hyper), beta1,
                                             beta2, eps, wd, ema_decay, ptr(sumsq_t), clip or 0.0, 1 if zero_grad else 0,
                                             stream_ptr()), "vaw_adamw_ema_step_dev")
        return
    bc1 = 1.0 - beta1 ** step
    bc2 = 1.0 - beta2 ** step
    check(L.lib().vaw_adamw_ema_step(ptr(p), ptr(g), ptr(m), ptr(v), ptr(ema), ptr(shadow), p.numel(), lr, beta1, beta2,
                                     eps, wd, bc1, bc2, ema_decay, ptr(sumsq_t), clip or 0.0, 1 if zero_grad else 0,
                                     stream_ptr()), "vaw_adamw_ema_step")


def ema_update(ema, src, decay):
    check(L.lib().vaw_ema_update(ptr(ema), ptr(src), ema.numel(), decay, stream_ptr()), "vaw_ema_update")


def cast_bf16(src, dst):
    check(L.lib().vaw_cast_bf16(ptr(src), ptr(dst), src.numel(), stream_ptr()), "vaw_cast_bf16")


def cast_colsum_plan(M, N, ld_src, ld_dst, src_addr, dst_addr, colsum_addr):
    p = L.CastColsumLaunch()
    rc = L.lib().vaw_cast_colsum_plan(M, N, ld_src, ld_dst, src_addr, dst_addr, colsum_addr, C.byref(p))
    return p if rc == 0 else None


def cast_colsum(src, ld_src, dst, ld_dst, M, N, colsum_out, beta=0.0):
    check(L.lib().vaw_cast_colsum_bf16(src, ld_src, dst, ld_dst, M, N, colsum_out, beta, stream_ptr()), "vaw_cast_colsum_bf16")


def silu_bwd(x, dy, dx, dx_bf16=None):
    check(L.lib().vaw_silu_bwd_cast(ptr(x), ptr(dy), ptr(dx), ptr(dx_bf16), dx.numel(), stream_ptr()), "vaw_silu_bwd_cast")


def uncast_bf16(src, dst, scale=1.0):
    check(L.lib().vaw_uncast_bf16(ptr(src), ptr(dst), src.numel(), float(scale), stream_ptr()), "vaw_uncast_bf16")


def gn_plan(gn_pass, dt, B, HW, C, G=32):
    p = L.GnLaunch()
    check(L.lib().vaw_gn_plan(gn_pass, dt, B, HW, C, G, L.C.byref(p)), "vaw_gn_plan")
    return p


def groupnorm_apply(dt, x, mean, rstd, gamma, beta, scale, shift, film_ld, silu, y, B, HW, C, G=32):
    check(L.lib().vaw_groupnorm_apply(dt, x, mean, rstd, gamma, beta, scale or None, shift or None, film_ld, 1 if silu else 0, y,
                                      B, HW, C, G, stream_ptr()), "vaw_groupnorm_apply")


def dropout_pack(dt, mask, M, C):
    bits = torch.empty(L.lib().vaw_dropout_bits_words(M * C), device=mask.device, dtype=torch.int32)
    check(L.lib().vaw_dropout_pack(dt, ptr(mask), ptr(bits), M, C, stream_ptr()), "vaw_dropout_pack")
    return bits


def dropout_bits(dt, x, bits, keep_scale, y, n, backward=False):
    fn = L.lib().vaw_dropout_bits_bwd if backward else L.lib().vaw_dropout_bits_fwd
    check(fn(dt, x, ptr(bits), keep_scale, y, n, stream_ptr()), "vaw_dropout_bits_bwd" if backward else "vaw_dropout_bits_fwd")


KSMALLEST_MAX = 16
WITHIN_MAX_RADII = 4


def _features(what, *ts):
    need_cuda(*ts)
    for t in ts:
        if t.dtype != torch.float32 or t.dim() != 2 or not t.is_contiguous() or t.shape[0] < 1 or t.shape[1] < 1:
            raise ValueError(f"{what}: features must be non-empty contiguous float32 [N, D] tensors, got {t.dtype} {tuple(t.shape)}")
        if t.shape[1] != ts[0].shape[1]:
            raise ValueError(f"{what}: feature widths differ: {ts[0].shape[1]} and {t.shape[1]}")


def _per_row(what, name, t, rows, cols=None, dtype=torch.float32):
    need_cuda(t)
    want = (rows,) if cols is None else (rows, cols)
    if t.dtype != dtype or tuple(t.shape) != want or not t.is_contiguous():
        raise ValueError(f"{what}: {name} must be a contiguous {dtype} tensor of shape {want}, got {t.dtype} {tuple(t.shape)}")


def row_sqnorms(x):
    _features("row_sqnorms", x)
    out = torch.empty(x.shape[0], device=x.device, dtype=torch.float32)
# ... 186 lines not shown
```

variance-aware-weight_amd/optim.py:

```python
import torch

from . import ops
from .flat import FlatModule


class FusedAdamW(torch.optim.Optimizer):
    def __init__(self, model, lr=1e-3, betas=(0.9, 0.999), eps=1e-8, weight_decay=1e-2):
        inner = getattr(model, "module", model)
        if not isinstance(inner, FlatModule):
            raise TypeError("FusedAdamW needs a vaw_amd FlatModule (e.g. vaw_amd.DiT); use torch.optim.AdamW otherwise")
        inner.ensure_flat()
        self.model = inner
        super().__init__(inner._flat_params, dict(lr=lr, betas=tuple(betas), eps=eps, weight_decay=weight_decay))
        n = inner._flat_n_train
        dev = inner._flat.device
        self.zero = getattr(inner, "_zero", None)
        if self.zero is not None:
            self._chunks = self.zero.owned_chunks()
            n = sum(hi - lo for lo, hi in self._chunks)
            self._ema_shard = self._ema_frozen = None
        self.exp_avg = torch.zeros(n, device=dev, dtype=torch.float32)
        self.exp_avg_sq = torch.zeros(n, device=dev, dtype=torch.float32)
        self._sumsq = torch.zeros(1, device=dev, dtype=torch.float32)
        self.step_count = 0
        self.ema_model, self.ema_decay = None, 0.0
        self.max_grad_norm = None
        self._flat_ptr = inner._flat.data_ptr()
        self.device_hyper = None
        self._hyper_host = None

    def enable_device_hyper(self):
        dev = self.model._flat.device
        self.device_hyper = torch.zeros(4, device=dev, dtype=torch.float32)
        self._hyper_host = torch.zeros(4, dtype=torch.float32).pin_memory() if dev.type == "cuda" else torch.zeros(4)

    def prepare_step(self):
        grp = self.param_groups[0]
        self.step_count += 1
        b1, b2 = grp["betas"]
        self._hyper_host[0] = grp["lr"]
        self._hyper_host[1] = 1.0 - b1 ** self.step_count
        self._hyper_host[2] = 1.0 - b2 ** self.step_count
        self.device_hyper.copy_(self._hyper_host, non_blocking=True)

    def attach_ema(self, ema_model, decay):
        e = getattr(ema_model, "module", ema_model)
        if not isinstance(e, FlatModule):
            raise TypeError("attach_ema needs a FlatModule EMA copy")
        e.ensure_flat()
        if e._flat_offsets != self.model._flat_offsets:
            raise ValueError("EMA model layout differs from the trained model")
        self.ema_model, self.ema_decay = e, float(decay)

    def attach_ema_sharded(self, decay, ema_model=None):
        assert self.zero is not None
        import torch.distributed as dist
        n = self.model._flat_n_train
        full = self.model._flat[:n].clone()
        if self.zero.rank == 0 and ema_model is not None:
            e = getattr(ema_model, "module", ema_model)
            e.ensure_flat()
            full.copy_(e._flat[:n])
        dist.broadcast(full, src=0, group=self.zero.pg)
        self._ema_shard = torch.cat([full[lo:hi] for lo, hi in self._chunks]).clone()
        self.ema_decay = float(decay)
        self._ema_frozen = None
        if ema_model is not None:
            e = getattr(ema_model, "module", ema_model)
            if e._flat.numel() > n:
                self._ema_frozen = e

    def _step_sharded(self):
        m, z, grp = self.model, self.zero, self.param_groups[0]
        m.ensure_flat()
        if m._flat.data_ptr() != self._flat_ptr:
            raise RuntimeError("the model's flat buffer was rebuilt (moved device / deep-copied) after the optimizer was created")
        g = m.flat_grads()
        z.wait_gathers()
        if self.device_hyper is None:
            self.step_count += 1
        clip = self.max_grad_norm
        if clip:
            for i, (lo, hi) in enumerate(self._chunks):
                ops.sumsq(g[lo:hi], self._sumsq, accumulate=i > 0)
            import torch.distributed as dist
            dist.all_reduce(self._sumsq, group=z.pg)
        shadow = m._flat_shadow
        off = 0
        for lo, hi in self._chunks:
            k = hi - lo
            ops.adamw_ema_step(m._flat[lo:hi], g[lo:hi], self.exp_avg[off:off + k], self.exp_avg_sq[off:off + k],
                               None if self._ema_shard is None else self._ema_shard[off:off + k],
                               None if shadow is None else shadow[lo:hi], grp["lr"], grp["betas"][0], grp["betas"][1], grp["eps"],
                               grp["weight_decay"], self.step_count, self.ema_decay, self._sumsq if clip else None, clip, False,
                               hyper=self.device_hyper)
            off += k
        if shadow is not None and not getattr(m, "_fp8", False):
            self._sync_f32_read_params()
            z.all_gather_chunks(shadow)
            self.master_stale = m._master_stale = True
        else:
            z.all_gather_chunks(m._flat)
            if shadow is not None:
                z.wait_gathers()
        if self._ema_shard is not None and self._ema_frozen is not None:
            n = m._flat_n_train
            ops.ema_update(self._ema_frozen._flat[n:], m._flat[n:], self.ema_decay)
        if shadow is None or not getattr(m, "_fp8", False):
            m.mark_shadow_fresh()
        else:
            m.mark_weights_changed()
        self.ema_done_in_step = self._ema_shard is not None

    def _sync_f32_read_params(self):
        import torch.distributed as dist
        m, z = self.model, self.zero
        hot = getattr(self, "_hot", None)
        if hot is None:
            emb = {n + ".weight" for n, mod in m.named_modules() if isinstance(mod, torch.nn.Embedding)}
            idx = [torch.arange(o, o + k) for n, p in zip(m._flat_names, m._flat_params) if (p.dim() == 1 or n in emb)
                   for o, k in [m._flat_offsets[n]]]
            idx = torch.cat(idx) if idx else torch.zeros(0, dtype=torch.long)
            own = torch.zeros(idx.numel(), dtype=torch.bool)
            for lo, hi in self._chunks:
                own |= (idx >= lo) & (idx < hi)
            dev = m._flat.device
            hot = self._hot = (idx.to(dev), own.to(dev))
        idx, own = hot
        if idx.numel() == 0:
            return
        vals = torch.where(own, m._flat[idx], torch.zeros((), device=idx.device))
        dist.all_reduce(vals, group=z.pg)
        m._flat[idx] = vals

    def consolidate(self):
        if self.zero is not None and getattr(self, "master_stale", False):
            self.zero.wait_gathers()
            self.zero.all_gather_chunks(self.model._flat, async_stream=False)
            self.master_stale = self.model._master_stale = False

    def consolidate_ema(self, ema_model):
        import torch.distributed as dist
        z = self.zero
        e = getattr(ema_model, "module", ema_model) if ema_model is not None else None
        full = torch.empty(self.model._flat_n_train, device=self.model._flat.device, dtype=torch.float32)
        off = 0
        for lo, hi in self._chunks:
            full[lo:hi] = self._ema_shard[off:off + hi - lo]
            off += hi - lo
        z.wait_gathers()
        z.all_gather_chunks(full, async_stream=False)
        if e is not None:
            e.ensure_flat()
            e._flat[: full.numel()].copy_(full)
            e.mark_weights_changed()

    def _gathered_moments(self):
        outs = []
        for shard in (self.exp_avg, self.exp_avg_sq):
            full = torch.zeros(self.model._flat_n_train, device=shard.device, dtype=torch.float32)
            off = 0
            for lo, hi in self._chunks:
                full[lo:hi] = shard[off:off + hi - lo]
                off += hi - lo
            self.zero.all_gather_chunks(full, async_stream=False)
            outs.append(full)
        return outs

    @torch.no_grad()
    def step(self, closure=None):
        assert closure is None
        if self.zero is not None:
            return self._step_sharded()
        m = self.model
        if getattr(m, "_zero", None) is not None:
            raise RuntimeError("this FusedAdamW was built BEFORE the model was wrapped with shard_optimizer=True: build the optimizer "
                               "after vaw_amd.DistributedDataParallel(model, shard_optimizer=True)")
        m.ensure_flat()
        if m._flat.data_ptr() != self._flat_ptr:
            raise RuntimeError("the model's flat buffer was rebuilt (moved device / deep-copied) after the optimizer was created")
        g = m.flat_grads()
        grp = self.param_groups[0]
        if self.device_hyper is None:
            self.step_count += 1
        n = m._flat_n_train
        clip = self.max_grad_norm
        if clip:
            ops.sumsq(g, self._sumsq)
        ema_flat = None
        if self.ema_model is not None:
            self.ema_model.ensure_flat()
            ema_flat = self.ema_model._flat
        shadow = m._flat_shadow
        ops.adamw_ema_step(m._flat[:n], g, self.exp_avg, self.exp_avg_sq, None if ema_flat is None else ema_flat[:n],
                           None if shadow is None else shadow[:n], grp["lr"], grp["betas"][0], grp["betas"][1], grp["eps"],
                           grp["weight_decay"], self.step_count, self.ema_decay, self._sumsq if clip else None, clip, False,
                           hyper=self.device_hyper)
        if ema_flat is not None and ema_flat.numel() > n:
            ops.ema_update(ema_flat[n:], m._flat[n:], self.ema_decay)
        m.mark_shadow_fresh()
        if self.ema_model is not None:
            self.ema_model.mark_weights_changed()
        self.ema_done_in_step = ema_flat is not None

    def zero_grad(self, set_to_none=True):
        self.model.zero_grad_flat()

    def _ckpt_params(self):
        m = self.model
        return [(n, p, n in m._flat_offsets and m._flat_offsets[n][0] < m._flat_n_train and p.requires_grad)
                for n, p in m.named_parameters()]

    def _moment_view(self, buf, name, p):
        m = self.model
        o, k = m._flat_offsets[name]
        return m._view_as_param(buf[o:o + k], p, m._flat_cl[name])

    def state_dict(self):
        self.model.ensure_flat()
        grp = {k: v for k, v in self.param_groups[0].items() if k != "params"}
        entries = self._ckpt_params()
        grp["params"] = list(range(len(entries)))
        state = {}
        if self.step_count > 0:
            exp_avg, exp_avg_sq = self._gathered_moments() if self.zero is not None else (self.exp_avg, self.exp_avg_sq)
            for i, (n, p, trainable) in enumerate(entries):
                if trainable:
                    state[i] = {"step": torch.tensor(float(self.step_count)),
                                "exp_avg": self._moment_view(exp_avg, n, p).contiguous().clone(),
                                "exp_avg_sq": self._moment_view(exp_avg_sq, n, p).contiguous().clone()}
        return {"state": state, "param_groups": [grp]}

    def load_state_dict(self, sd):
        self.model.ensure_flat()
        if self.zero is not None:
            shards = (self.exp_avg, self.exp_avg_sq)
            n = self.model._flat_n_train
            self.exp_avg, self.exp_avg_sq = (torch.zeros(n, device=shards[0].device) for _ in range(2))
            try:
                self._load_state_dict_full(sd)
                full = (self.exp_avg, self.exp_avg_sq)
            finally:
                self.exp_avg, self.exp_avg_sq = shards
            for shard, f in zip(shards, full):
                shard.copy_(torch.cat([f[lo:hi] for lo, hi in self._chunks]))
            return
        self._load_state_dict_full(sd)

    def _load_state_dict_full(self, sd):
        flat = sd.get("vaw_flat")
        if flat is not None:
            self.exp_avg.copy_(flat["exp_avg"])
            self.exp_avg_sq.copy_(flat["exp_avg_sq"])
            self.step_count = int(flat["step"])
        else:
            state = sd.get("state", {})
            entries = self._ckpt_params()
            groups = sd.get("param_groups", [])
            n_saved = sum(len(g.get("params", [])) for g in groups)
            if state and n_saved != len(entries):
                raise ValueError(f"optimizer state covers {n_saved} parameters, the model has {len(entries)}")
            steps = set()
            self.exp_avg.zero_()
            self.exp_avg_sq.zero_()
            for i, (n, p, trainable) in enumerate(entries):
                st = state.get(i, state.get(str(i)))
                if st is None:
                    continue
                if not trainable:
                    raise ValueError(f"optimizer state for frozen parameter {n}")
                if tuple(st["exp_avg"].shape) != tuple(p.shape):
                    raise ValueError(f"optimizer state of {n}: shape {tuple(st['exp_avg'].shape)} != {tuple(p.shape)}")
                self._moment_view(self.exp_avg, n, p).copy_(st["exp_avg"])
                self._moment_view(self.exp_avg_sq, n, p).copy_(st["exp_avg_sq"])
                steps.add(int(float(st["step"])))
            if len(steps) > 1:
                raise ValueError(f"per-parameter step counts differ ({sorted(steps)}): the fused kernel keeps one")
            self.step_count = steps.pop() if steps else 0
        for g_new, g_old in zip(self.param_groups, sd["param_groups"]):
            for k in ("lr", "betas", "eps", "weight_decay", "initial_lr"):
# ... 3 lines not shown
```

variance-aware-weight_amd/trainer.py:

```python
from contextlib import nullcontext

import torch
import torch.nn as nn

from . import _lib, dist_util, ops
from .flat import FlatModule
from .optim import FusedAdamW


def ema(source, target, decay):
    s, t = getattr(source, "module", source), getattr(target, "module", target)
    with torch.no_grad():
        if isinstance(s, FlatModule) and isinstance(t, FlatModule):
            s.ensure_flat(); t.ensure_flat()
            if s._flat_offsets == t._flat_offsets and s._flat.is_cuda and not list(s.buffers()):
                ops.ema_update(t._flat, s._flat, decay)
                t.mark_weights_changed()
                return
        src, dst = source.state_dict(), target.state_dict()
        for k in src:
            dst[k].data.copy_(dst[k].data * decay + src[k].data * (1 - decay))
        if isinstance(t, FlatModule) and getattr(t, "_flat", None) is not None:
            t.mark_weights_changed()

# ... 51 lines not shown
        self.schedule_sampler, self._device_sampler = None, False
        name = getattr(args, "schedule_sampler", None)
        if name and name != "uniform":
            from .resample import create_named_schedule_sampler
            self.schedule_sampler = create_named_schedule_sampler(name, diffusion, device=device)
            self._device_sampler = hasattr(self.schedule_sampler, "ring")
            if getattr(args, "hip_graph", False) and not self._device_sampler:
                raise ValueError("args.schedule_sampler updates its history on the host every step: not with args.hip_graph")
        self._graph, self._graph_calls, self._gin, self._gout = None, 0, None, None
        hg = getattr(args, "hip_graph", False)
        self._graph_auto = hg == "auto"
        self._use_graph = bool(hg)
        if self._use_graph:
            why = ("needs vaw_amd.FusedAdamW" if not self._fused else "not with DDP (args.parallel)" if args.parallel else
                   "not with grad_accumulation > 1" if max(1, args.grad_accumulation) > 1 else
                   "not with args.cpu_rng" if self._cpu_rng else "needs a CUDA device" if torch.device(device).type != "cuda" else
                   "the model draws its label-drop mask on the host every step (UNet drop_label_prob > 0)"
                   if getattr(inner, "host_rng_in_forward", False) else None)
            if why and self._graph_auto:
                self._use_graph = False
            elif why:
                raise ValueError(f"args.hip_graph: {why}")
            else:
                optimizer.enable_device_hyper()

    def _get_next_batch(self):
        try:
            images, labels = next(self.datalooper)
        except StopIteration:
            self.datalooper = iter(self.train_loader)
            return self._get_next_batch()
        return (images.to(self.device, non_blocking=True),
                labels.to(self.device, non_blocking=True) if self.args.class_cond else None)

    def _compute_loss(self, images, labels, features, accum=None):
        model_kwargs = {"y": labels} if self.args.class_cond else {}
        extra = {"accum": accum} if accum is not None and self._fused_means else {}
        if self._cpu_rng and not self._device_sampler:
            noise = torch.randn(images.shape).to(images.device)
            t = torch.randint(0, self.diffusion.num_timesteps, (images.shape[0],)).to(images.device)
            return self.diffusion.training_losses(self.model, images, features, t=t, model_kwargs=model_kwargs, noise=noise, **extra)
        if self.schedule_sampler is not None:
            noise = torch.randn(images.shape).to(images.device) if self._cpu_rng else None
            t, w = self.schedule_sampler.sample(images.shape[0], images.device)
            terms = self.diffusion.training_losses(self.model, images, features, t=t, model_kwargs=model_kwargs, noise=noise)
            self.schedule_sampler.update_with_local_losses(t, terms["loss"].detach())
            terms = dict(terms)
            terms["loss"] = terms["loss"] * w
            return terms
        return self.diffusion.training_losses(self.model, images, features, model_kwargs=model_kwargs, **extra)

    def _micro_step(self, images, labels, accum, cpu_rng, divide):
        a = self.args
        fused = self._step_fused and images.is_cuda
        if fused and a.in_chans == 4 and self.schedule_sampler is None and self._fused_latent:
            mean, _ = torch.chunk(images, 2, dim=1)
            model_kwargs = {"y": labels} if a.class_cond else {}
            if cpu_rng:
                eps = torch.randn(mean.shape).to(mean.device)
                model_kwargs = dict(model_kwargs=model_kwargs, noise=torch.randn(mean.shape).to(mean.device),
                                    t=torch.randint(0, self.diffusion.num_timesteps, (mean.shape[0],)).to(mean.device))
            else:
                eps = torch.randn_like(mean)
                model_kwargs = dict(model_kwargs=model_kwargs)
            loss_dict = self.diffusion.training_losses_fused(self.model, images, a.latent_scale, eps, accum=accum, **model_kwargs)
        else:
            if a.in_chans == 4:
                images = sample_from_latent(images, a.latent_scale, cpu_rng)
            loss_dict = self._compute_loss(images, labels, None, accum if fused else None)
        if "loss_mean" in loss_dict:
            loss = loss_dict["loss_mean"]
            torch.autograd.backward(loss, ops.one_like(loss))
            return loss.detach(), loss_dict["mse_mean"]
        loss = loss_dict["loss"].mean()
        if divide:
            loss = loss / accum
        loss.backward()
        ld = loss.detach()
        if "mse" not in loss_dict:
            return ld, torch.zeros_like(ld)
        md = loss_dict["mse"].detach().mean()
        return ld, (md / accum if divide else md)

    def _apply_gradient_clipping(self):
        if self.args.grad_clip:
            if self._fused:
                self.optimizer.max_grad_norm = float(self.args.grad_clip)
            else:
                nn.utils.clip_grad_norm_(self.model.parameters(), self.args.grad_clip)

    def consolidate(self):
        if self._zero:
            self.optimizer.consolidate()
            if getattr(self.optimizer, "_ema_shard", None) is not None:
                self.optimizer.consolidate_ema(self.ema_model)

    def _update_ema(self):
        if self._zero:
            return
        if dist_util.is_main_process() and self.ema_model is not None:
            if self._fused and getattr(self.optimizer, "ema_done_in_step", False):
                return
            ema(self.model, self.ema_model, self.args.ema_decay)

    def _graph_body(self, images, labels):
        loss, mse = self._micro_step(images, labels, 1, False, False)
        self._apply_gradient_clipping()
        self.optimizer.step()
        self.optimizer.zero_grad()
        return loss, mse

    def eager_from_now_on(self):
        if self._use_graph:
            self._graph, self._gin, self._gout = None, None, None
            self._graph_calls = -(1 << 60)

    def _train_step_graph(self, step):
        a = self.args
        self.model.train()
        images, labels = self._get_next_batch()
        self.optimizer.prepare_step()
        self._graph_calls += 1
        if self._graph is None and self._graph_calls <= 2:
            if self._graph_auto and self._graph_calls == 2:
                import time
                e0, e1 = torch.cuda.Event(enable_timing=True), torch.cuda.Event(enable_timing=True)
                torch.cuda.synchronize()
                t0 = time.perf_counter()
                e0.record()
                total, mse = self._graph_body(images, labels)
                e1.record()
                host_ms = 1e3 * (time.perf_counter() - t0)
                torch.cuda.synchronize()
                self.graph_decision = dict(host_ms=host_ms, gpu_ms=e0.elapsed_time(e1))
                if host_ms < 0.7 * self.graph_decision["gpu_ms"]:
                    self._graph_calls = -(1 << 60)
            else:
                total, mse = self._graph_body(images, labels)
        elif self._graph_calls < 0:
            total, mse = self._graph_body(images, labels)
        else:
            if self._graph is None:
                self._gin = (images.clone(), None if labels is None else labels.clone())
                torch.cuda.synchronize()
                g = torch.cuda.CUDAGraph()
                with torch.cuda.graph(g):
                    self._gout = self._graph_body(*self._gin)
                self._graph = g
            else:
                self._gin[0].copy_(images, non_blocking=True)
                if labels is not None:
                    self._gin[1].copy_(labels, non_blocking=True)
            self._graph.replay()
            total, mse = self._gout
        self.scheduler.step()
        if dist_util.is_main_process():
            self._update_ema()
        self.last_mse = mse
        if dist_util.is_main_process() and self.pbar is not None:
            self.pbar.update(1)
        if getattr(a, "defer_loss_sync", False):
            return total
        total_f = float(total.item())
        if dist_util.is_main_process() and self.pbar is not None:
            self.pbar.set_postfix(mse=f"{float(mse.item()):.4f}")
        return total_f

    def train_step(self, step):
        if self._use_graph:
            return self._train_step_graph(step)
        a = self.args
        self.model.train()
        if a.parallel:
            self.train_loader.sampler.set_epoch(step)
        accum = max(1, a.grad_accumulation)
        total, mse_avg = None, None
        for i in range(accum):
            images, labels = self._get_next_batch()
            if a.parallel and accum > 1 and i < accum - 1:
                ctx = self.model.no_sync()
            else:
                ctx = nullcontext()
            with ctx:
                ld, md = self._micro_step(images, labels, accum, self._cpu_rng, True)
            total = ld if total is None else total + ld
            mse_avg = md if mse_avg is None else mse_avg + md
            if (i + 1) % accum == 0:
                self._apply_gradient_clipping()
                self.optimizer.step()
                self.optimizer.zero_grad()
        self.scheduler.step()
        if dist_util.is_main_process():
            self._update_ema()
        self.last_mse = mse_avg
        if getattr(a, "defer_loss_sync", False):
            if dist_util.is_main_process() and self.pbar is not None:
                self.pbar.update(1)
            return total
        total_f = float(total.item())
        if dist_util.is_main_process() and self.pbar is not None:
            self.pbar.update(1)
            self.pbar.set_postfix(mse=f"{float(mse_avg.item()):.4f}")
        return total_f
```

Before: 21030 images/sec.

## Overlap early AdamW update on side stream with backward; widen group fixup

Adds an optional early optimizer path: once the parameters outside a late range have final gradients, a hook launches a lean AdamW+EMA kernel for those ranges on a side stream, overlapping it with the rest of backward. The late range is updated afterwards in the normal step, which then waits on an event. It also replaces the grouped wgrad split-K fixup kernel with a wider variant that uses more blocks and batched slab loads. The early path is gated by an environment variable that defaults to off, so by default only the wider fixup kernel runs.

Result: no change. 20990 images/sec (-0.2%).

```diff
diff --git a/include/vaw_hip.h b/include/vaw_hip.h
--- a/include/vaw_hip.h
+++ b/include/vaw_hip.h
@@ -201,6 +201,8 @@
 int vaw_wgrad_grouped(vaw_dtype dt, int n_problems, const vaw_wgrad_problem* problems, int64_t K, float beta, void* desc_dev,
                       int upload, float* workspace, int64_t workspace_floats, vaw_stream stream);
 void vaw_debug_wgrad_engine(int mode);
+void vaw_debug_group_fixup(int mode);
+int vaw_wgrad_grouped_four_wave(vaw_dtype dt, int n_problems, const vaw_wgrad_problem* problems);
 
 int64_t vaw_fp8_quantize_workspace_floats(void);
 int vaw_fp8_quantize(vaw_dtype src_dt, vaw_dtype dst_format, const void* src, int64_t R, int64_t C, int64_t ld, void* q, int64_t ldq,
@@ -504,6 +506,11 @@
 int vaw_adamw_ema_step_dev(float* p, float* g, float* m, float* v, float* ema, void* shadow_bf16, int64_t n,
                            const float* hyper, float beta1, float beta2, float eps, float weight_decay, float ema_decay,
                            const float* sumsq, float clip_max_norm, int zero_grad, vaw_stream stream);
+int vaw_adamw_ema_step_lean(float* p, float* g, float* m, float* v, float* ema, void* shadow_bf16, int64_t n,
+                            const float* hyper, float lr, float beta1, float beta2, float eps, float weight_decay, float bc1,
+                            float bc2, float ema_decay, const float* sumsq, float clip_max_norm, int zero_grad, vaw_stream stream);
+void vaw_debug_adamw_early(int mode);
+int vaw_adamw_early_enabled(void);
 int vaw_ema_update(float* ema, const float* src, int64_t n, float decay, vaw_stream stream);
 int vaw_cast_bf16(const float* src, void* dst, int64_t n, vaw_stream stream);
 typedef struct {
diff --git a/variance-aware-weight_amd/_lib.py b/variance-aware-weight_amd/_lib.py
--- a/variance-aware-weight_amd/_lib.py
+++ b/variance-aware-weight_amd/_lib.py
@@ -181,6 +181,9 @@
     "vaw_sumsq": [_p, _l, _p, _i, _p, _p],
     "vaw_adamw_ema_step_dev": [_p, _p, _p, _p, _p, _p, _l, _p, _f, _f, _f, _f, _f, _p, _f, _i, _p],
     "vaw_adamw_ema_step": [_p, _p, _p, _p, _p, _p, _l, _f, _f, _f, _f, _f, _f, _f, _f, _p, _f, _i, _p],
+    "vaw_adamw_ema_step_lean": [_p, _p, _p, _p, _p, _p, _l, _p, _f, _f, _f, _f, _f, _f, _f, _f, _p, _f, _i, _p],
+    "vaw_wgrad_grouped_four_wave": [_i, _i, _p],
+    "vaw_adamw_early_enabled": [],
     "vaw_ema_update": [_p, _p, _l, _f, _p],
     "vaw_cast_bf16": [_p, _p, _l, _p],
     "vaw_uncast_bf16": [_p, _p, _l, _f, _p],
@@ -292,6 +295,11 @@
         if hasattr(L, "vaw_debug_wgrad_engine"):
             L.vaw_debug_wgrad_engine.argtypes = [_i]
             L.vaw_debug_wgrad_engine.restype = None
+        if hasattr(L, "vaw_debug_adamw_early"):
+            L.vaw_debug_adamw_early.argtypes = [_i]
+            L.vaw_debug_adamw_early.restype = None
+            L.vaw_debug_group_fixup.argtypes = [_i]
+            L.vaw_debug_group_fixup.restype = None
         L.vaw_debug_cu_hog.argtypes = [_i, _i, _p]
         L.vaw_debug_cu_hog.restype = _i
         _lib = L
@@ -303,7 +311,7 @@
                                    "vaw_sumsq_workspace_floats", "vaw_groupnorm_workspace_floats", "vaw_wgrad_grouped_desc_bytes",
                                    "vaw_conv3x3_wgrad_small_workspace_floats", "vaw_row_bwd_workspace_floats",
                                    "vaw_fp8_quantize_workspace_floats", "vaw_p8_set_reserved_cus", "vaw_debug_wgrad_engine", "vaw_reduce_rows_batched_desc_bytes", "vaw_fp8_quantize_batched_desc_bytes",
-                                   "vaw_gemm_default_knobs", "vaw_dropout_bits_words", "vaw_pairwise_workspace_bytes", "vaw_rk_partial_count",
+                                   "vaw_gemm_default_knobs", "vaw_debug_adamw_early", "vaw_debug_group_fixup", "vaw_dropout_bits_words", "vaw_pairwise_workspace_bytes", "vaw_rk_partial_count",
                                    "vaw_pairwise_polysum_workspace_bytes", "vaw_pairwise_count_workspace_bytes"])
 
 
diff --git a/variance-aware-weight_amd/csrc/elementwise.hip b/variance-aware-weight_amd/csrc/elementwise.hip
--- a/variance-aware-weight_amd/csrc/elementwise.hip
+++ b/variance-aware-weight_amd/csrc/elementwise.hip
@@ -882,6 +882,89 @@
         if (a.zero_grad) g[i] = 0.f;
     }
 }
+
+#define ADAM_LEAN_U 2
+static_assert(ADAM_U % ADAM_LEAN_U == 0, "a tile is a whole number of in-flight groups");
+__global__ void __launch_bounds__(256, 6)
+adamw_ema_lean_kernel(float* __restrict__ p, float* __restrict__ g, float* __restrict__ m, float* __restrict__ v,
+                      float* __restrict__ ema, bf16_t* __restrict__ shadow, int64_t n, const float* __restrict__ sumsq, AdamArgs a,
+                      const float* __restrict__ hyper) {
+    if (hyper) {
+        a.lr = hyper[0];
+        a.bc1 = hyper[1];
+        a.bc2_sqrt = sqrtf(hyper[2]);
+    }
+    float gs = 1.f;
+    if (a.clip > 0.f) {
+        const float coef = a.clip / (sqrtf(*sumsq) + 1e-6f);
+        gs = coef < 1.f ? coef : 1.f;
+    }
+    const int64_t n4 = n / 4;
+    const bool has_ema = ema != nullptr;
+    constexpr int U = ADAM_LEAN_U;
+    constexpr int64_t TILE = (int64_t)ADAM_U * 256;
+    const int64_t n_tiles = n4 / TILE;
+    const unsigned l0 = 16u * threadIdx.x;
+    auto at = [](auto* base, unsigned byte_off) { return reinterpret_cast<decltype(base)>(reinterpret_cast<char*>(base) + byte_off); };
+    for (int64_t t = blockIdx.x; t < n_tiles; t += gridDim.x) {
+#pragma unroll 1
+        for (int h = 0; h < ADAM_U / U; ++h) {
+            const int64_t tb0 = 4 * (t * TILE + h * (U * 256));
+            const int64_t tb = ((int64_t)__builtin_amdgcn_readfirstlane((int)(tb0 >> 32)) << 32) |
+                               (uint32_t)__builtin_amdgcn_readfirstlane((int)(uint32_t)tb0);
+            float *pt = p + tb, *gt = g + tb, *mt = m + tb, *vt = v + tb, *et = has_ema ? ema + tb : nullptr;
+            unsigned li = l0;
+            asm volatile("" : "+v"(li));
+            f32x4 pv[U], gv[U], mv[U], vv[U], ev[U];
+#pragma unroll
+            for (int u = 0; u < U; ++u) {
+                const unsigned i = li + 4096u * u;
+                pv[u] = nt_load4(at(pt, i)); gv[u] = nt_load4(at(gt, i)); mv[u] = nt_load4(at(mt, i)); vv[u] = nt_load4(at(vt, i));
+                ev[u] = has_ema ? nt_load4(at(et, i)) : f32x4{0, 0, 0, 0};
+            }
+#pragma unroll
+            for (int u = 0; u < U; ++u) {
+                const unsigned i = li + 4096u * u;
+#pragma unroll
+                for (int j = 0; j < 4; ++j) {
+                    float pj = pv[u][j], gj = gv[u][j], mj = mv[u][j], vj = vv[u][j], ej = ev[u][j];
+                    adam_one(pj, gj, mj, vj, ej, has_ema, gs, a);
+                    pv[u][j] = pj; mv[u][j] = mj; vv[u][j] = vj; ev[u][j] = ej;
+                }
+                __builtin_nontemporal_store(pv[u], reinterpret_cast<f32x4*>(at(pt, i)));
+                __builtin_nontemporal_store(mv[u], reinterpret_cast<f32x4*>(at(mt, i)));
+                __builtin_nontemporal_store(vv[u], reinterpret_cast<f32x4*>(at(vt, i)));
+                if (has_ema) __builtin_nontemporal_store(ev[u], reinterpret_cast<f32x4*>(at(et, i)));
+                if (shadow) store4(at(shadow + tb, i / 2), pv[u]);
+                if (a.zero_grad) store4(at(gt, i), f32x4{0, 0, 0, 0});
+            }
+        }
+    }
+    for (int64_t i = n_tiles * TILE + blockIdx.x * (int64_t)blockDim.x + threadIdx.x; i < n4; i += (int64_t)gridDim.x * blockDim.x) {
+        f32x4 pv = load4(p + 4 * i), gv = load4(g + 4 * i), mv = load4(m + 4 * i), vv = load4(v + 4 * i);
+        f32x4 ev = has_ema ? load4(ema + 4 * i) : f32x4{0, 0, 0, 0};
+#pragma unroll
+        for (int j = 0; j < 4; ++j) {
+            float pj = pv[j], gj = gv[j], mj = mv[j], vj = vv[j], ej = ev[j];
+            adam_one(pj, gj, mj, vj, ej, has_ema, gs, a);
+            pv[j] = pj; mv[j] = mj; vv[j] = vj; ev[j] = ej;
+        }
+        store4(p + 4 * i, pv);
+        store4(m + 4 * i, mv);
+        store4(v + 4 * i, vv);
+        if (has_ema) store4(ema + 4 * i, ev);
+        if (shadow) store4(shadow + 4 * i, pv);
+        if (a.zero_grad) store4(g + 4 * i, f32x4{0, 0, 0, 0});
+    }
+    for (int64_t i = n4 * 4 + blockIdx.x * (int64_t)blockDim.x + threadIdx.x; i < n; i += (int64_t)gridDim.x * blockDim.x) {
+        float pv = p[i], gv = g[i], mv = m[i], vv = v[i], ev = has_ema ? ema[i] : 0.f;
+        adam_one(pv, gv, mv, vv, ev, has_ema, gs, a);
+        p[i] = pv; m[i] = mv; v[i] = vv;
+        if (has_ema) ema[i] = ev;
+        if (shadow) shadow[i] = (bf16_t)pv;
+        if (a.zero_grad) g[i] = 0.f;
+    }
+}
 static inline int adam_grid(int64_t n) {
     const int64_t tiles = n / 4 / (ADAM_U * 256);
     const int64_t cap = 256 * 8;
@@ -913,6 +996,38 @@
     AdamArgs a{0.f, beta1, beta2, eps, weight_decay, 1.f, 1.f, ema_decay, clip_max_norm, zero_grad};
     adamw_ema_kernel<<<adam_grid(n), 256, 0, (hipStream_t)stream>>>(p, g, m, v, ema, (bf16_t*)shadow_bf16, n, sumsq, a, hyper);
     VAW_CHECK_LAUNCH("adamw_ema_dev");
+    return VAW_OK;
+}
+
+#define ADAMW_EARLY_DEFAULT 0
+static int g_adamw_early = -2;
+extern "C" int vaw_adamw_early_enabled(void) {
+    if (g_adamw_early == -2) {
+        const char* e = getenv("VAW_ADAMW_EARLY");
+        const int m = e ? atoi(e) : -1;
+        g_adamw_early = (m == 0 || m == 1) ? m : -1;
+    }
+    return g_adamw_early < 0 ? ADAMW_EARLY_DEFAULT : g_adamw_early;
+}
+extern "C" void vaw_debug_adamw_early(int mode) { g_adamw_early = (mode == 0 || mode == 1) ? mode : -1; }
+
+int vaw_p8_cus_available();
+extern "C" int vaw_adamw_ema_step_lean(float* p, float* g, float* m, float* v, float* ema, void* shadow_bf16, int64_t n,
+                                       const float* hyper, float lr, float beta1, float beta2, float eps, float weight_decay,
+                                       float bc1, float bc2, float ema_decay, const float* sumsq, float clip_max_norm,
+                                       int zero_grad, vaw_stream stream) {
+    VAW_CHECK_ARG(n > 0, "adamw_lean: n<=0");
+    VAW_CHECK_ARG((((uintptr_t)p | (uintptr_t)g | (uintptr_t)m | (uintptr_t)v | (uintptr_t)ema) & 15) == 0 &&
+                      ((uintptr_t)shadow_bf16 & 7) == 0, "adamw_lean: buffers (range starts) must be 16-byte aligned");
+    VAW_CHECK_ARG(p && g && m && v, "adamw_lean: null buffer");
+    VAW_CHECK_ARG(clip_max_norm <= 0.f || sumsq != nullptr, "adamw_lean: clip needs sumsq");
+    AdamArgs a{lr, beta1, beta2, eps, weight_decay, bc1, sqrtf(bc2), ema_decay, clip_max_norm, zero_grad};
+    if (hyper) { a.lr = 0.f; a.bc1 = 1.f; a.bc2_sqrt = 1.f; }
+    const int64_t tiles = n / 4 / (ADAM_U * 256);
+    const int cus = vaw_p8_cus_available();
+    const int grid = (int)(tiles < 1 ? 1 : (tiles > cus ? cus : tiles));
+    adamw_ema_lean_kernel<<<grid, 256, 0, (hipStream_t)stream>>>(p, g, m, v, ema, (bf16_t*)shadow_bf16, n, sumsq, a, hyper);
+    VAW_CHECK_LAUNCH("adamw_ema_lean");
     return VAW_OK;
 }
 
diff --git a/variance-aware-weight_amd/csrc/gemm_p8.hip b/variance-aware-weight_amd/csrc/gemm_p8.hip
--- a/variance-aware-weight_amd/csrc/gemm_p8.hip
+++ b/variance-aware-weight_amd/csrc/gemm_p8.hip
@@ -102,6 +102,24 @@
 }
 extern "C" void vaw_debug_wgrad_engine(int mode) { g_wgrad_engine = (mode == 0 || mode == 1) ? mode : -1; }
 
+static int g_group_fixup_ref = 0;
+extern "C" void vaw_debug_group_fixup(int mode) { g_group_fixup_ref = mode == 1 ? 1 : 0; }
+
+static int wgrad_group_ntw(int n_problems, const vaw_wgrad_problem* problems) {
+    bool all192 = true, any_not256 = false;
+    for (int i = 0; i < n_problems; ++i) {
+        all192 = all192 && problems[i].N % 192 == 0;
+        any_not256 = any_not256 || problems[i].N % 256 != 0;
+    }
+    return (all192 && any_not256) ? 3 : 4;
+}
+
+extern "C" int vaw_wgrad_grouped_four_wave(vaw_dtype dt, int n_problems, const vaw_wgrad_problem* problems) {
+    if (dt != VAW_BF16 || n_problems <= 0 || !problems || wgrad_group_ntw(n_problems, problems) != 4) return 0;
+    const int eng = wgrad_engine();
+    return (eng == 1 || (eng < 0 && G4_BY_SHAPE)) ? 1 : 0;
+}
+
 extern "C" int64_t vaw_wgrad_grouped_desc_bytes(int n_problems) { return (int64_t)n_problems * (int64_t)sizeof(P8Prob); }
 
 extern "C" int vaw_wgrad_grouped(vaw_dtype dt, int n_problems, const vaw_wgrad_problem* problems, int64_t K, float beta,
@@ -110,7 +128,6 @@
     const bool f8 = dt == VAW_FP8 || dt == VAW_BF8;
     const int kt = f8 ? 128 : 64;
     VAW_CHECK_ARG(n_problems > 0 && problems && desc_dev && K > 0 && K % kt == 0, "wgrad_grouped: bad arguments (K %% %d)", kt);
-    bool all192 = true, any_not256 = false;
     for (int i = 0; i < n_problems; ++i) {
         const vaw_wgrad_problem& q = problems[i];
         VAW_CHECK_ARG(q.dy && q.x && q.dw && q.M >= 16 && q.N >= 16 && q.M % 8 == 0 && q.N % 8 == 0, "wgrad_grouped: problem %d: M, N", i);
@@ -120,10 +137,8 @@
                            "wgrad_grouped: problem %d: leading dimensions", i);
         VAW_CHECK_ARG((((uintptr_t)q.dy | (uintptr_t)q.x | (uintptr_t)q.dw) & 15) == 0, "wgrad_grouped: problem %d: alignment", i);
         VAW_CHECK_ARG(q.M < (1 << 30) && q.N < (1 << 30), "wgrad_grouped: problem %d too large", i);
-        all192 = all192 && q.N % 192 == 0;
-        any_not256 = any_not256 || q.N % 256 != 0;
-    }
-    const int ntw = (all192 && any_not256) ? 3 : 4, bn = 64 * ntw;
+    }
+    const int ntw = wgrad_group_ntw(n_problems, problems), bn = 64 * ntw;
     static thread_local std::vector<P8Prob> host;
     host.resize(n_problems);
     int64_t t_total = 0;
@@ -187,9 +202,12 @@
         if (eng == 1 || (eng < 0 && G4_BY_SHAPE)) vaw_g4_launch_group(nk, grid, e, (const P8Prob*)desc_dev, grp, s);
         else p8_launch_group<4>(nk, grid, e, (const P8Prob*)desc_dev, grp, s);
     } else p8_launch_group<3>(nk, grid, e, (const P8Prob*)desc_dev, grp, s);
-    if (grp.t_rem > 0) {
+    if (grp.t_rem > 0 && g_group_fixup_ref) {
         if (ntw == 4) p8_group_fixup_kernel<256><<<grp.t_rem * 8, 256, 0, s>>>((const P8Prob*)desc_dev, grp, beta);
         else p8_group_fixup_kernel<192><<<grp.t_rem * 8, 256, 0, s>>>((const P8Prob*)desc_dev, grp, beta);
+    } else if (grp.t_rem > 0) {
+        if (ntw == 4) p8_group_fixup_wide_kernel<256><<<grp.t_rem * 32, 256, 0, s>>>((const P8Prob*)desc_dev, grp, beta);
+        else p8_group_fixup_wide_kernel<192><<<grp.t_rem * 32, 256, 0, s>>>((const P8Prob*)desc_dev, grp, beta);
     }
     VAW_CHECK_LAUNCH("wgrad_grouped");
     return VAW_OK;
diff --git a/variance-aware-weight_amd/csrc/gemm_p8_kernel.h b/variance-aware-weight_amd/csrc/gemm_p8_kernel.h
--- a/variance-aware-weight_amd/csrc/gemm_p8_kernel.h
+++ b/variance-aware-weight_amd/csrc/gemm_p8_kernel.h
@@ -874,6 +874,40 @@
     }
 }
 
+template <int BN>
+__global__ void __launch_bounds__(256) p8_group_fixup_wide_kernel(const P8Prob* __restrict__ probs, P8Group grp, float beta) {
+    const int r = blockIdx.x >> 5, band = blockIdx.x & 31, g = grp.t_full + r;
+    int pi = 0;
+    while (pi + 1 < grp.n_prob && probs[pi + 1].tile0 <= g) ++pi;
+    const P8Prob pr = probs[pi];
+    const int tile = g - pr.tile0, tm = tile / pr.tiles_n, tn = tile - tm * pr.tiles_n;
+    const int64_t m0 = (int64_t)tm * P8_BM + 8 * band, n0 = (int64_t)tn * BN;
+    constexpr int C4 = BN / 4, CH = 8;
+    const int64_t sp_stride = (int64_t)grp.t_rem * (P8_BM * BN);
+    for (int i = threadIdx.x; i < 8 * C4; i += blockDim.x) {
+        const int row = i / C4, c4 = (i - row * C4) * 4;
+        const int64_t m = m0 + row, n = n0 + c4;
+        if (m >= pr.M || n >= pr.N) continue;
+        const float* s0 = grp.slab + (int64_t)r * (P8_BM * BN) + (int64_t)(8 * band + row) * BN + c4;
+        float* c = pr.c + m * pr.ldc + n;
+        f32x4 cv = {0, 0, 0, 0};
+        if (beta != 0.f) cv = load4(c);
+        f32x4 acc = {0, 0, 0, 0};
+        for (int sp = 0; sp < grp.n_split; sp += CH) {
+            f32x4 v[CH];
+#pragma unroll
+            for (int k = 0; k < CH; ++k)
+                if (sp + k < grp.n_split) v[k] = load4(s0 + (sp + k) * sp_stride);
+#pragma unroll
+            for (int k = 0; k < CH; ++k)
+                if (sp + k < grp.n_split) acc += v[k];
+        }
+        acc *= pr.alpha * (pr.scale_a ? *pr.scale_a : 1.f) * (pr.scale_b ? *pr.scale_b : 1.f);
+        if (beta != 0.f) acc += beta * cv;
+        store4(c, acc);
+    }
+}
+
 struct P8Launch {
     const bf16_t *a, *b;
     int64_t lda, ldb;
diff --git a/variance-aware-weight_amd/dit.py b/variance-aware-weight_amd/dit.py
--- a/variance-aware-weight_amd/dit.py
+++ b/variance-aware-weight_amd/dit.py
@@ -236,6 +236,7 @@
         self.set_activation_checkpointing(activation_checkpointing)
         self._ckpt_debug_hook = None
         self.grad_ready_hook = None
+        self.params_final_hook = None
         self.defer_wgrad = True
 
     def initialize_weights(self):
@@ -320,6 +321,10 @@
             lo = [(0, cut_w), (we, cut_b), (be, first[0])] if wo < bo else [(0, cut_b), (be, cut_w), (we, first[0])]
             b[0] = [r for r in lo if r[1] > r[0]]
         return b
+
+    def early_late_range(self):
+        self.ensure_flat()
+        return self._flat_offsets["blocks.0.attn.qkv.weight"][0], self._flat_offsets["final_layer.linear.weight"][0]
 
     def _ada_split_block(self):
         return self.depth // 2 if self.depth >= 4 else None
@@ -627,6 +632,9 @@
             hook(Lyr + 1)
         pending = []
         group_cut = Lyr // 2 if (hook and Lyr >= 4) else 0
+        early = self.params_final_hook
+        if not (early is not None and hook is None and not only_dx and not ckpt and not fp8 and defer and Lyr > 0):
+            early = None
 
         def fold_bias(blocks, qkv_too):
             key = (blocks[0], blocks[-1], self._gbase, qkv_too)
@@ -643,9 +651,7 @@
             grp = ent[0]
             grp.launch(beta)
 
-        def flush():
-            if not pending:
-                return
+        def group_of():
             key = (pending[0], pending[-1], self._gbase)
             grp = ws.wgrad_groups.get(key)
             if grp is None:
@@ -661,8 +667,14 @@
                                                 (pre + "attn.proj.", b["dy1"], b["ao"], D, D), (pre + "attn.qkv.", b["dqkv"], b["xm"], 3 * D, D)):
                         probs.append((ptr(dy), ptr(x), self._g(name + "weight"), Nw, Kw, Nw, Kw, Kw))
                 grp = ws.wgrad_groups[key] = ops.WgradGroup(probs, M, dout.device)
-            grp.launch((L.BF8 if self.fp8_grad_format == "e5m2" else L.FP8) if fp8 else dt, beta)
-            fold_bias(list(pending), True)
+            return grp
+
+        def flush(fold=True):
+            if not pending:
+                return
+            group_of().launch((L.BF8 if self.fp8_grad_format == "e5m2" else L.FP8) if fp8 else dt, beta)
+            if fold:
+                fold_bias(list(pending), True)
             if hook:
                 for l in pending:
                     hook(l + 1)
@@ -714,7 +726,7 @@
                 pass
             elif defer:
                 pending.append(l)
-                if ckpt or l == group_cut:
+                if ckpt or (l == group_cut and early is None):
                     pending.reverse()
                     flush()
             else:
@@ -727,7 +739,12 @@
                     self._adaln_wgrad(dt, ws, r0, ld - r0, B, beta)
                     hook("ada_hi")
         pending.reverse()
-        flush()
+        if early is not None and not (len(pending) == Lyr and group_of().four_wave(dt)):
+            early = None
+        if early is not None:
+            fold_bias(list(pending), True)
+        else:
+            flush()
         if dt == BF16 and fuse_tail and Lyr:
             dx0 = ptr(ws.dao)
         elif dt == BF16:
@@ -761,6 +778,9 @@
             ops.cast_bf16(ws.dh1, ws.dh1_a)
         dh1_a = ptr(ws.dh1_a) if dt == BF16 else ptr(ws.dh1)
         self._wgrad(dt, "t_embedder.mlp.0.", dh1_a, ptr(ws.tfreq), D, 256, ws.Bk, beta)
+        if early is not None:
+            early()
+            flush(fold=False)
         self.attach_grads()
         if fp8:
             ws.calib_bwd = True
diff --git a/variance-aware-weight_amd/flat.py b/variance-aware-weight_amd/flat.py
--- a/variance-aware-weight_amd/flat.py
+++ b/variance-aware-weight_amd/flat.py
@@ -97,7 +97,7 @@
         memo[id(self)] = new
         import copy
         skip = {"_flat", "_flat_grad", "_flat_shadow", "_flat_params"}
-        fresh = {"_ws": dict, "_ws_cur": lambda: None, "_adesc": lambda: None, "_tape": list, "_fp8_w": dict, "_fp8_epoch": lambda: None, "_fp8_wstates": lambda: None, "_fp8_wgroup": lambda: None, "_zero": lambda: None, "grad_ready_hook": lambda: None}
+        fresh = {"_ws": dict, "_ws_cur": lambda: None, "_adesc": lambda: None, "_tape": list, "_fp8_w": dict, "_fp8_epoch": lambda: None, "_fp8_wstates": lambda: None, "_fp8_wgroup": lambda: None, "_zero": lambda: None, "grad_ready_hook": lambda: None, "params_final_hook": lambda: None}
         for k, v in self.__dict__.items():
             new.__dict__[k] = None if k in skip else fresh[k]() if k in fresh else copy.deepcopy(v, memo)
         new._flat_dirty = True
diff --git a/variance-aware-weight_amd/ops.py b/variance-aware-weight_amd/ops.py
--- a/variance-aware-weight_amd/ops.py
+++ b/variance-aware-weight_amd/ops.py
@@ -752,6 +752,22 @@
                         float(sum(es * (p.M + p.N) * self.K + 4 * p.M * p.N * (2 if beta else 1) for p in self.table)))
 
 
+    def four_wave(self, dt):
+        return bool(L.lib().vaw_wgrad_grouped_four_wave(dt, self.n, C.cast(self.table, C.c_void_p)))
+
+
+def group_fixup(mode):
+    L.lib().vaw_debug_group_fixup(int(mode))
+
+
+def adamw_early(mode):
+    L.lib().vaw_debug_adamw_early(int(mode))
+
+
+def adamw_early_enabled():
+    return bool(L.lib().vaw_adamw_early_enabled())
+
+
 def wgrad_engine(mode):
     L.lib().vaw_debug_wgrad_engine(int(mode))
 
@@ -1050,7 +1066,14 @@
     check(L.lib().vaw_sumsq(ptr(g), g.numel(), ptr(out), 1 if accumulate else 0, ptr(ws), stream_ptr()), "vaw_sumsq")
 
 
-def adamw_ema_step(p, g, m, v, ema, shadow, lr, beta1, beta2, eps, wd, step, ema_decay, sumsq_t, clip, zero_grad, hyper=None):
+def adamw_ema_step(p, g, m, v, ema, shadow, lr, beta1, beta2, eps, wd, step, ema_decay, sumsq_t, clip, zero_grad, hyper=None,
+                   lean=False):
+    if lean:
+        bc1, bc2 = (1.0, 1.0) if hyper is not None else (1.0 - beta1 ** step, 1.0 - beta2 ** step)
+        check(L.lib().vaw_adamw_ema_step_lean(ptr(p), ptr(g), ptr(m), ptr(v), ptr(ema), ptr(shadow), p.numel(), ptr(hyper), lr, beta1,
+                                              beta2, eps, wd, bc1, bc2, ema_decay, ptr(sumsq_t), clip or 0.0, 1 if zero_grad else 0,
+                                              stream_ptr()), "vaw_adamw_ema_step_lean")
+        return
     if hyper is not None:
         check(L.lib().vaw_adamw_ema_step_dev(ptr(p), ptr(g), ptr(m), ptr(v), ptr(ema), ptr(shadow), p.numel(), ptr(hyper), beta1,
                                              beta2, eps, wd, ema_decay, ptr(sumsq_t), clip or 0.0, 1 if zero_grad else 0,
diff --git a/variance-aware-weight_amd/optim.py b/variance-aware-weight_amd/optim.py
--- a/variance-aware-weight_amd/optim.py
+++ b/variance-aware-weight_amd/optim.py
@@ -2,6 +2,21 @@
 
 from . import ops
 from .flat import FlatModule
+
+
+def early_plan(n_train, late):
+    lo, hi = int(late[0]), int(late[1])
+    if not (0 <= lo < hi <= n_train):
+        raise ValueError(f"early_plan: late range [{lo}, {hi}) outside [0, {n_train})")
+    early = [(a, b) for a, b in ((0, lo), (hi, n_train)) if b > a]
+    for a, _ in early + [(lo, hi)]:
+        if a % 4:
+            raise ValueError(f"early_plan: range start {a} is not a multiple of 4 elements")
+    return early, [(lo, hi)]
+
+
+def early_eligible(*, enabled, sharded, listener, max_grad_norm, steps_now, capturing):
+    return bool(enabled and not sharded and not listener and not max_grad_norm and steps_now and not capturing)
 
 
 class FusedAdamW(torch.optim.Optimizer):
@@ -28,6 +43,52 @@
         self._flat_ptr = inner._flat.data_ptr()
         self.device_hyper = None
         self._hyper_host = None
+        self.early_launches = 0
+        self._early_plan = None
+        self._early_stream = None
+        self._early_done = None
+        self._early_scalars = None
+
+    def arm_early(self, steps_now=True, max_grad_norm=None):
+        m = self.model
+        ok = hasattr(m, "params_final_hook") and hasattr(m, "early_late_range") and m._flat.is_cuda and early_eligible(
+            enabled=ops.adamw_early_enabled(), sharded=self.zero is not None or getattr(m, "_zero", None) is not None,
+            listener=m.grad_ready_hook is not None, max_grad_norm=max_grad_norm or self.max_grad_norm, steps_now=steps_now,
+            capturing=torch.cuda.is_current_stream_capturing())
+        if hasattr(m, "params_final_hook"):
+            m.params_final_hook = self._early_launch if ok else None
+        return ok
+
+    def _update_range(self, lo, hi, lr, step, lean):
+        m, grp = self.model, self.param_groups[0]
+        ema_flat = None if self.ema_model is None else self.ema_model._flat
+        shadow = m._flat_shadow
+        ops.adamw_ema_step(m._flat[lo:hi], m._flat_grad[lo:hi], self.exp_avg[lo:hi], self.exp_avg_sq[lo:hi],
+                           None if ema_flat is None else ema_flat[lo:hi], None if shadow is None else shadow[lo:hi], lr,
+                           grp["betas"][0], grp["betas"][1], grp["eps"], grp["weight_decay"], step, self.ema_decay, None, None, False,
+                           hyper=self.device_hyper, lean=lean)
+
+    def _early_launch(self):
+        m = self.model
+        m.params_final_hook = None
+        if torch.cuda.is_current_stream_capturing() or m._flat.data_ptr() != self._flat_ptr or m._flat_grad is None:
+            return
+        if self._early_plan is None:
+            self._early_plan = early_plan(m._flat_n_train, m.early_late_range())
+            self._early_stream = torch.cuda.Stream(device=m._flat.device)
+            self._early_done = torch.cuda.Event()
+        if self.ema_model is not None:
+            self.ema_model.ensure_flat()
+        lr = self.param_groups[0]["lr"]
+        step = self.step_count if self.device_hyper is not None else self.step_count + 1
+        side = self._early_stream
+        side.wait_stream(torch.cuda.current_stream())
+        with torch.cuda.stream(side):
+            for lo, hi in self._early_plan[0]:
+                self._update_range(lo, hi, lr, step, True)
+            self._early_done.record(side)
+        self._early_scalars = (lr, step)
+        self.early_launches += 1
 
     def enable_device_hyper(self):
         dev = self.model._flat.device
@@ -184,7 +245,12 @@
         if self.device_hyper is None:
             self.step_count += 1
         n = m._flat_n_train
+        if hasattr(m, "params_final_hook"):
+            m.params_final_hook = None
+        early, self._early_scalars = self._early_scalars, None
         clip = self.max_grad_norm
+        if early is not None and clip:
+            raise RuntimeError("FusedAdamW: max_grad_norm was set after arm_early() let a step start its update early")
         if clip:
             ops.sumsq(g, self._sumsq)
         ema_flat = None
@@ -192,10 +258,17 @@
             self.ema_model.ensure_flat()
             ema_flat = self.ema_model._flat
         shadow = m._flat_shadow
-        ops.adamw_ema_step(m._flat[:n], g, self.exp_avg, self.exp_avg_sq, None if ema_flat is None else ema_flat[:n],
-                           None if shadow is None else shadow[:n], grp["lr"], grp["betas"][0], grp["betas"][1], grp["eps"],
-                           grp["weight_decay"], self.step_count, self.ema_decay, self._sumsq if clip else None, clip, False,
-                           hyper=self.device_hyper)
+        if early is not None:
+            lr, step = early
+            assert step == self.step_count
+            for lo, hi in self._early_plan[1]:
+                self._update_range(lo, hi, lr, step, False)
+            torch.cuda.current_stream().wait_event(self._early_done)
+        else:
+            ops.adamw_ema_step(m._flat[:n], g, self.exp_avg, self.exp_avg_sq, None if ema_flat is None else ema_flat[:n],
+                               None if shadow is None else shadow[:n], grp["lr"], grp["betas"][0], grp["betas"][1], grp["eps"],
+                               grp["weight_decay"], self.step_count, self.ema_decay, self._sumsq if clip else None, clip, False,
+                               hyper=self.device_hyper)
         if ema_flat is not None and ema_flat.numel() > n:
             ops.ema_update(ema_flat[n:], m._flat[n:], self.ema_decay)
         m.mark_shadow_fresh()
diff --git a/variance-aware-weight_amd/trainer.py b/variance-aware-weight_amd/trainer.py
--- a/variance-aware-weight_amd/trainer.py
+++ b/variance-aware-weight_amd/trainer.py
@@ -157,6 +157,10 @@
         md = loss_dict["mse"].detach().mean()
         return ld, (md / accum if divide else md)
 
+    def _arm_early(self, steps_now):
+        if self._fused and not self.args.parallel:
+            self.optimizer.arm_early(steps_now=steps_now, max_grad_norm=self.args.grad_clip)
+
     def _apply_gradient_clipping(self):
         if self.args.grad_clip:
             if self._fused:
@@ -179,6 +183,7 @@
             ema(self.model, self.ema_model, self.args.ema_decay)
 
     def _graph_body(self, images, labels):
+        self._arm_early(True)
         loss, mse = self._micro_step(images, labels, 1, False, False)
         self._apply_gradient_clipping()
         self.optimizer.step()
@@ -256,6 +261,7 @@
                 ctx = self.model.no_sync()
             else:
                 ctx = nullcontext()
+            self._arm_early(accum == 1)
             with ctx:
                 ld, md = self._micro_step(images, labels, accum, self._cpu_rng, True)
             total = ld if total is None else total + ld
```
